# kscalelabs/minppo

Measured on NVIDIA B200. Metric: learner transitions/sec (GAE+PPO epochs), higher is better.
Workload: dtype bf16 tensor-core GEMMs (fp32 accumulate), fp32 elsewhere

## Files before the change

### minppo_b200/csrc/common.cuh

```cuda
#pragma once

#include <cuda.h>
#include <cuda_bf16.h>
#include <cuda_runtime.h>
#include <stdint.h>

namespace minppo {

#define MINPPO_DEVINL __device__ __forceinline__

MINPPO_DEVINL uint32_t smem_u32(const void* p) {
  return static_cast<uint32_t>(__cvta_generic_to_shared(p));
}

MINPPO_DEVINL uint32_t lane_id() { return threadIdx.x & 31u; }

MINPPO_DEVINL bool elect_one() {
  uint32_t pred = 0;
  asm volatile(
      "{\n\t.reg .pred P;\n\t"
      "elect.sync _|P, 0xffffffff;\n\t"
      "selp.u32 %0, 1, 0, P;\n\t}\n"
      : "=r"(pred));
  return pred != 0;
}

MINPPO_DEVINL float warp_sum(float v) {
#pragma unroll
  for (int o = 16; o > 0; o >>= 1) v += __shfl_xor_sync(0xffffffffu, v, o);
  return v;
}

MINPPO_DEVINL void griddep_wait() { asm volatile("griddepcontrol.wait;" ::: "memory"); }
MINPPO_DEVINL void griddep_launch() { asm volatile("griddepcontrol.launch_dependents;" ::: "memory"); }

MINPPO_DEVINL void mbar_init(uint64_t* bar, uint32_t count) {
  asm volatile("mbarrier.init.shared::cta.b64 [%0], %1;" ::"r"(smem_u32(bar)), "r"(count));
}
MINPPO_DEVINL void fence_mbar_init() {
  asm volatile("fence.mbarrier_init.release.cluster;" ::: "memory");
}
MINPPO_DEVINL void mbar_arrive(uint64_t* bar) {
  asm volatile("mbarrier.arrive.shared::cta.b64 _, [%0];" ::"r"(smem_u32(bar)) : "memory");
}
MINPPO_DEVINL void mbar_arrive_expect_tx(uint64_t* bar, uint32_t bytes) {
  asm volatile("mbarrier.arrive.expect_tx.shared::cta.b64 _, [%0], %1;" ::"r"(smem_u32(bar)),
               "r"(bytes)
               : "memory");
}
#ifndef MINPPO_TRY_WAIT_HINT_NS
#define MINPPO_TRY_WAIT_HINT_NS 1000000u
#endif
MINPPO_DEVINL bool mbar_try_wait(uint64_t* bar, uint32_t parity) {
  uint32_t ok;
  asm volatile(
      "{\n\t.reg .pred P;\n\t"
      "mbarrier.try_wait.parity.shared::cta.b64 P, [%1], %2, %3;\n\t"
      "selp.u32 %0, 1, 0, P;\n\t}\n"
      : "=r"(ok)
      : "r"(smem_u32(bar)), "r"(parity), "r"(MINPPO_TRY_WAIT_HINT_NS)
      : "memory");
  return ok != 0;
}
#ifndef MINPPO_WAIT_SLEEP_NS
#define MINPPO_WAIT_SLEEP_NS 0
#endif
template <bool POLITE = true>
MINPPO_DEVINL void mbar_wait(uint64_t* bar, uint32_t parity) {
  if (mbar_try_wait(bar, parity)) return;
  const long long t0 = clock64();
  for (;;) {
#pragma unroll 1
    for (int i = 0; i < 64; ++i) {
      if (mbar_try_wait(bar, parity)) return;
#if MINPPO_WAIT_SLEEP_NS
      if (POLITE) asm volatile("nanosleep.u32 %0;" ::"r"(static_cast<uint32_t>(MINPPO_WAIT_SLEEP_NS)));
#endif
    }
    if (clock64() - t0 > 4000000000LL) __trap();
  }
}

#ifndef MINPPO_MMA_SPIN
#define MINPPO_MMA_SPIN 0
#endif
MINPPO_DEVINL void mbar_wait_spin(uint64_t* bar, uint32_t parity) {
#if MINPPO_MMA_SPIN
  const uint32_t addr = smem_u32(bar);
  const long long t0 = clock64();
  for (;;) {
#pragma unroll 1
    for (int i = 0; i < 32; ++i) {
      uint32_t ok;
      asm volatile(
          "{\n\t.reg .pred P;\n\t"
          "mbarrier.test_wait.parity.shared::cta.b64 P, [%1], %2;\n\t"
          "selp.u32 %0, 1, 0, P;\n\t}\n"
          : "=r"(ok)
          : "r"(addr), "r"(parity)
          : "memory");
      if (ok) return;
    }
    if (clock64() - t0 > 4000000000LL) __trap();
  }
#else
  mbar_wait<false>(bar, parity);
#endif
}

MINPPO_DEVINL void fence_proxy_async_smem() {
  asm volatile("fence.proxy.async.shared::cta;" ::: "memory");
}

MINPPO_DEVINL void cp_async_16(uint32_t smem_dst, const void* gsrc) {
  asm volatile("cp.async.cg.shared.global [%0], [%1], 16;" ::"r"(smem_dst), "l"(gsrc) : "memory");
}
MINPPO_DEVINL void cp_async_commit() { asm volatile("cp.async.commit_group;" ::: "memory"); }
template <int N>
MINPPO_DEVINL void cp_async_wait() {
  asm volatile("cp.async.wait_group %0;" ::"n"(N) : "memory");
}

MINPPO_DEVINL void tma_prefetch_desc(const CUtensorMap* m) {
  asm volatile("prefetch.tensormap [%0];" ::"l"(reinterpret_cast<uint64_t>(m)) : "memory");
}
MINPPO_DEVINL void tma_load_2d(uint32_t smem_dst, const CUtensorMap* m, uint64_t* bar, int c0, int c1) {
  asm volatile(
      "cp.async.bulk.tensor.2d.shared::cluster.global.mbarrier::complete_tx::bytes"
      " [%0], [%1, {%3, %4}], [%2];"
      ::"r"(smem_dst), "l"(reinterpret_cast<uint64_t>(m)), "r"(smem_u32(bar)), "r"(c0), "r"(c1)
      : "memory");
}

MINPPO_DEVINL void tma_store_2d(uint32_t smem_src, const CUtensorMap* m, int c0, int c1) {
  asm volatile("cp.async.bulk.tensor.2d.global.shared::cta.bulk_group [%0, {%2, %3}], [%1];" ::"l"(
                   reinterpret_cast<uint64_t>(m)),
               "r"(smem_src), "r"(c0), "r"(c1)
               : "memory");
}
MINPPO_DEVINL void tma_store_3d(uint32_t smem_src, const CUtensorMap* m, int c0, int c1, int c2) {
  asm volatile("cp.async.bulk.tensor.3d.global.shared::cta.bulk_group [%0, {%2, %3, %4}], [%1];" ::"l"(
                   reinterpret_cast<uint64_t>(m)),
               "r"(smem_src), "r"(c0), "r"(c1), "r"(c2)
               : "memory");
}
MINPPO_DEVINL void bulk_store_1d(void* gdst, uint32_t smem_src, uint32_t bytes) {
  asm volatile("cp.async.bulk.global.shared::cta.bulk_group [%0], [%1], %2;" ::"l"(gdst), "r"(smem_src), "r"(bytes) : "memory");
}
MINPPO_DEVINL void sts32(uint32_t addr, float v) { asm volatile("st.shared.f32 [%0], %1;" ::"r"(addr), "f"(v) : "memory"); }
MINPPO_DEVINL void tma_store_commit() { asm volatile("cp.async.bulk.commit_group;" ::: "memory"); }
MINPPO_DEVINL void tma_store_wait_read0() { asm volatile("cp.async.bulk.wait_group.read 0;" ::: "memory"); }
MINPPO_DEVINL void tma_store_wait_all0() { asm volatile("cp.async.bulk.wait_group 0;" ::: "memory"); }
MINPPO_DEVINL void fence_proxy_async_global() { asm volatile("fence.proxy.async.global;" ::: "memory"); }

MINPPO_DEVINL void sts128(uint32_t addr, uint4 v) {
  asm volatile("st.shared.v4.u32 [%0], {%1, %2, %3, %4};" ::"r"(addr), "r"(v.x), "r"(v.y), "r"(v.z), "r"(v.w) : "memory");
}
MINPPO_DEVINL uint4 lds128(uint32_t addr) {
  uint4 v;
  asm volatile("ld.shared.v4.u32 {%0, %1, %2, %3}, [%4];" : "=r"(v.x), "=r"(v.y), "=r"(v.z), "=r"(v.w) : "r"(addr));
  return v;
}

MINPPO_DEVINL void tmem_alloc(uint32_t* smem_dst, uint32_t ncols) {
  asm volatile("tcgen05.alloc.cta_group::1.sync.aligned.shared::cta.b32 [%0], %1;" ::"r"(smem_u32(smem_dst)),
               "r"(ncols)
               : "memory");
}
MINPPO_DEVINL void tmem_relinquish() {
  asm volatile("tcgen05.relinquish_alloc_permit.cta_group::1.sync.aligned;" ::: "memory");
}
MINPPO_DEVINL void tmem_dealloc(uint32_t taddr, uint32_t ncols) {
  asm volatile("tcgen05.dealloc.cta_group::1.sync.aligned.b32 %0, %1;" ::"r"(taddr), "r"(ncols) : "memory");
}
MINPPO_DEVINL void tc_fence_before() { asm volatile("tcgen05.fence::before_thread_sync;" ::: "memory"); }
MINPPO_DEVINL void tc_fence_after() { asm volatile("tcgen05.fence::after_thread_sync;" ::: "memory"); }

MINPPO_DEVINL void umma_bf16(uint32_t tmem_d, uint64_t desc_a, uint64_t desc_b, uint32_t idesc,
                             uint32_t accumulate) {
  asm volatile(
      "{\n\t.reg .pred p;\n\t"
      "setp.ne.b32 p, %4, 0;\n\t"
      "tcgen05.mma.cta_group::1.kind::f16 [%0], %1, %2, %3, p;\n\t}\n"
      ::"r"(tmem_d), "l"(desc_a), "l"(desc_b), "r"(idesc), "r"(accumulate)
      : "memory");
}
MINPPO_DEVINL void umma_commit(uint64_t* bar) {
  asm volatile("tcgen05.commit.cta_group::1.mbarrier::arrive::one.shared::cluster.b64 [%0];" ::"r"(smem_u32(bar))
               : "memory");
}

MINPPO_DEVINL void tmem_ld_32x32(uint32_t taddr, float (&v)[32]) {
  uint32_t* r = reinterpret_cast<uint32_t*>(v);
  asm volatile(
      "tcgen05.ld.sync.aligned.32x32b.x32.b32 "
      "{%0, %1, %2, %3, %4, %5, %6, %7, %8, %9, %10, %11, %12, %13, %14, %15, "
      "%16, %17, %18, %19, %20, %21, %22, %23, %24, %25, %26, %27, %28, %29, %30, %31}, [%32];"
      : "=r"(r[0]), "=r"(r[1]), "=r"(r[2]), "=r"(r[3]), "=r"(r[4]), "=r"(r[5]), "=r"(r[6]), "=r"(r[7]),
        "=r"(r[8]), "=r"(r[9]), "=r"(r[10]), "=r"(r[11]), "=r"(r[12]), "=r"(r[13]), "=r"(r[14]), "=r"(r[15]),
        "=r"(r[16]), "=r"(r[17]), "=r"(r[18]), "=r"(r[19]), "=r"(r[20]), "=r"(r[21]), "=r"(r[22]), "=r"(r[23]),
        "=r"(r[24]), "=r"(r[25]), "=r"(r[26]), "=r"(r[27]), "=r"(r[28]), "=r"(r[29]), "=r"(r[30]), "=r"(r[31])
      : "r"(taddr)
      : "memory");
}
MINPPO_DEVINL void tmem_ld_wait() { asm volatile("tcgen05.wait::ld.sync.aligned;" ::: "memory"); }

MINPPO_DEVINL uint64_t umma_smem_desc(uint32_t smem_addr, uint32_t lbo_bytes, uint32_t sbo_bytes) {
  uint64_t d = 0;
  d |= static_cast<uint64_t>((smem_addr & 0x3FFFFu) >> 4);
  d |= static_cast<uint64_t>((lbo_bytes >> 4) & 0x3FFFu) << 16;
  d |= static_cast<uint64_t>((sbo_bytes >> 4) & 0x3FFFu) << 32;
  d |= static_cast<uint64_t>(1) << 46;
  d |= static_cast<uint64_t>(2) << 61;
  return d;
}
MINPPO_DEVINL constexpr uint32_t umma_idesc_bf16(uint32_t M, uint32_t N, uint32_t a_mn_major,
                                                 uint32_t b_mn_major) {
  return (1u << 4)
         | (1u << 7)
         | (1u << 10)
         | (a_mn_major << 15)
         | (b_mn_major << 16)
         | ((N >> 3) << 17)
         | ((M >> 4) << 24);
}

MINPPO_DEVINL float fast_tanh(float x) {
  float y;
  asm("tanh.approx.f32 %0, %1;" : "=f"(y) : "f"(x));
  return y;
}
MINPPO_DEVINL float exp_tanh(float x) {
  float e, r;
  asm("ex2.approx.ftz.f32 %0, %1;" : "=f"(e) : "f"(x * 2.8853900817779268f));
  asm("rcp.approx.ftz.f32 %0, %1;" : "=f"(r) : "f"(e + 1.f));
  return fmaf(-2.f, r, 1.f);
}

MINPPO_DEVINL uint32_t pack_bf16x2(float lo, float hi) {
  __nv_bfloat162 h = __floats2bfloat162_rn(lo, hi);
  return *reinterpret_cast<uint32_t*>(&h);
}
MINPPO_DEVINL void split_bf16(float x, uint32_t& hi, uint32_t& lo) {
  const __nv_bfloat16 h = __float2bfloat16_rn(x);
  const __nv_bfloat16 l = __float2bfloat16_rn(x - __bfloat162float(h));
  hi = __bfloat16_as_ushort(h);
  lo = __bfloat16_as_ushort(l);
}
MINPPO_DEVINL uint32_t swp_off(int ap, int rr, int c) {
  return static_cast<uint32_t>((c >> 6) * (ap * 256) + rr * 128 + ((((c & 63) >> 3) ^ (rr & 7)) << 4) + (c & 7) * 2);
}
MINPPO_DEVINL float bf16_lo(uint32_t w) { return __uint_as_float(w << 16); }
MINPPO_DEVINL float bf16_hi(uint32_t w) { return __uint_as_float(w & 0xFFFF0000u); }

}
```

### minppo_b200/csrc/dwopt.cuh

```cuda
#pragma once

#include "opt_common.cuh"
#include "umma_gemm.cuh"

namespace minppo {

constexpr int DWOPT_THREADS = 512;

struct PeerXchg {
  char* base[MINPPO_MAX_RANKS];
  unsigned int* seq;
  int world, rank;
  int np;
  int two_phase;
  int ablate;
};
MINPPO_DEVINL float* px_stage(const PeerXchg& x, int r, unsigned int par, int q) {
  return reinterpret_cast<float*>(x.base[r]) + (static_cast<size_t>(par) * x.world + q) * x.np;
}
MINPPO_DEVINL float* px_result(const PeerXchg& x, int r, unsigned int par) {
  return reinterpret_cast<float*>(x.base[r]) + 2 * static_cast<size_t>(x.world) * x.np + static_cast<size_t>(x.world) * 256 +
         static_cast<size_t>(par) * x.np;
}
MINPPO_DEVINL float4 ld_sys_v4(const float* p) {
  float4 v;
  asm volatile("ld.relaxed.sys.global.v4.f32 {%0, %1, %2, %3}, [%4];" : "=f"(v.x), "=f"(v.y), "=f"(v.z), "=f"(v.w) : "l"(p) : "memory");
  return v;
}
MINPPO_DEVINL void st_sys_f32(float* p, float v) { asm volatile("st.relaxed.sys.global.f32 [%0], %1;" ::"l"(p), "f"(v) : "memory"); }
MINPPO_DEVINL void st_sys_v4(float* p, float4 v) {
  asm volatile("st.relaxed.sys.global.v4.f32 [%0], {%1, %2, %3, %4};" ::"l"(p), "f"(v.x), "f"(v.y), "f"(v.z), "f"(v.w) : "memory");
}
MINPPO_DEVINL unsigned int ld_relaxed_sys_u32(const unsigned int* p) {
  unsigned int v;
  asm volatile("ld.relaxed.sys.global.u32 %0, [%1];" : "=r"(v) : "l"(p) : "memory");
  return v;
}
MINPPO_DEVINL void ld_unit(const float* p, float (&v)[4]) {
  const uintptr_t a = reinterpret_cast<uintptr_t>(p);
  if ((a & 15u) == 0) { const float4 q = __ldcg(reinterpret_cast<const float4*>(p)); v[0] = q.x; v[1] = q.y; v[2] = q.z; v[3] = q.w; }
  else if ((a & 7u) == 0) {
    const float2 q0 = __ldcg(reinterpret_cast<const float2*>(p)), q1 = __ldcg(reinterpret_cast<const float2*>(p) + 1);
    v[0] = q0.x; v[1] = q0.y; v[2] = q1.x; v[3] = q1.y;
  } else {
#pragma unroll
    for (int e = 0; e < 4; ++e) v[e] = __ldcg(p + e);
  }
}
MINPPO_DEVINL void st_unit(float* p, const float (&v)[4]) {
  const uintptr_t a = reinterpret_cast<uintptr_t>(p);
  if ((a & 15u) == 0) *reinterpret_cast<float4*>(p) = make_float4(v[0], v[1], v[2], v[3]);
  else if ((a & 7u) == 0) { reinterpret_cast<float2*>(p)[0] = make_float2(v[0], v[1]); reinterpret_cast<float2*>(p)[1] = make_float2(v[2], v[3]); }
  else {
#pragma unroll
    for (int e = 0; e < 4; ++e) p[e] = v[e];
  }
}

struct alignas(64) DwOptParams {
  GemmParams gemm;
  OptArgs opt;
  int gemm_ctas;
  long long* trace;
  PeerXchg px;
  const int32_t* ridx_base;
  const int32_t* counts;
  int cap, EM;
  int padded;
  int losses_stride;
  int part_rows;
  int prefetch;
  const __nv_bfloat16* obs_img;
  int obs_ld;
  int step;
};

template <int NTHREADS_MAX = 1024>
MINPPO_DEVINL float block_sum_dyn(float v, float* scratch ) {
  const int nw = static_cast<int>(blockDim.x) >> 5;
  v = warp_sum(v);
  if ((threadIdx.x & 31) == 0) scratch[threadIdx.x >> 5] = v;
  __syncthreads();
  float s = 0.f;
  if (threadIdx.x < 32) {
    s = static_cast<int>(threadIdx.x) < nw ? scratch[threadIdx.x] : 0.f;
    s = warp_sum(s);
  }
  __syncthreads();
  return s;
}

template <int MAXU>
MINPPO_DEVINL void dwopt_body(const DwOptParams& p, int step, uint8_t* smem_raw, uint32_t ext_tmem, bool build_tab = true) {
  __shared__ float scratch[32];
  __shared__ float s_bcast[4];
  __shared__ LeafTab T;
  const OptArgs& a = p.opt;
  const int P = a.P;
  const int G = static_cast<int>(gridDim.x), NT = static_cast<int>(blockDim.x);
  const int32_t* row_count = p.padded ? p.counts + step : nullptr;
  const int32_t* next_ridx = (p.prefetch && step + 1 < p.EM) ? p.ridx_base + static_cast<size_t>(step + 1) * p.cap : nullptr;
  const int32_t* next_count = p.padded ? p.counts + step + 1 : nullptr;
  float* losses_out = a.losses_out ? a.losses_out + static_cast<size_t>(step) * p.losses_stride : nullptr;
  float* gnorm_out = a.gnorm_out ? a.gnorm_out + step : nullptr;
  const int b = static_cast<int>(blockIdx.x), t = static_cast<int>(threadIdx.x);
  const bool has_extra = p.gemm_ctas < G;
#define DW_STAMP(slot) do { if (p.trace && t == 0) p.trace[static_cast<size_t>(b) * 16 + (slot)] = clock64(); } while (0)
  float ss = 0.f;
  DW_STAMP(0);
  __shared__ unsigned int s_seq;
  __shared__ int s_dead;
  const bool px_on = p.px.world > 1;
  if (px_on && t == 0) {
    s_seq = __ldcg(p.px.seq) + 1u;
    s_dead = __ldcg(a.err_flag) != 0;
  }
  const bool gemm_cta = b < p.gemm_ctas;
  if (!gemm_cta) {
    if (build_tab) leaf_tab_build(T, a, t, NT);
    __syncthreads();
  }
  DW_STAMP(14);

  const bool scal_thread = t == NT - 1;
  int count = 0;
  float ent = a.entropy_const;
  auto scalars = [&]() {
    if (scal_thread && a.do_apply) {
      count = __ldcg(a.count);
      step_scalars(a, count, s_bcast[1], s_bcast[2], s_bcast[3]);
      if (b == 0 && losses_out) {
        for (int j = 0; j < a.A; ++j) ent += logf(fabsf(expf(__ldcg(a.params + a.off_logstd + j))));
      }
    }
  };

  if (gemm_cta) {
    auto idle_work = [&]() {
      if (build_tab) leaf_tab_build(T, a, t - GEMM_THREADS, NT - GEMM_THREADS);
      scalars();
      if (next_ridx) {
        const int HELPERS = NT - GEMM_THREADS;
        const int h = t - GEMM_THREADS;
        const int lines = (p.obs_ld * 2) >> 7;
        const int nrows = next_count ? min(p.cap, __ldcg(next_count)) : p.cap;
        for (int j = b * HELPERS + h; j < nrows * lines; j += p.gemm_ctas * HELPERS) {
          const char* row = reinterpret_cast<const char*>(p.obs_img + static_cast<size_t>(next_ridx[j / lines]) * p.obs_ld);
          asm volatile("prefetch.global.L2 [%0];" ::"l"(row + (j % lines) * 128));
        }
      }
    };
    umma_gemm_body<EPI_PARTIAL>(p.gemm, smem_raw, p.trace ? p.trace + static_cast<size_t>(b) * 16 : nullptr, idle_work, ext_tmem,
                                p.ridx_base + static_cast<size_t>(step) * p.cap, row_count);
  } else {
    scalars();
    griddep_wait();
    if (t == 0) griddep_launch();
    const int e = b - p.gemm_ctas, ne = G - p.gemm_ctas;
    const int live_tiles = row_count ? (max(__ldcg(row_count), 0) + p.part_rows - 1) / p.part_rows : 0x7fffffff;
    ss = reduce_leaves<false>(a, T, e * NT + t, ne * NT, live_tiles);
  }
  DW_STAMP(1);
  grid_barrier(a.barrier, a.err_flag);
  DW_STAMP(2);

  int n_units = 0;
  for (int l = 0; l < T.nleaves; ++l)
    if (T.leaf[l].late) n_units += T.size[l] >> 2;
  const int GT_ = G * NT;
  const bool fast = n_units <= GT_ * MAXU;
  const int gtid = b * NT + t;
  float4 g4[MAXU];
  float pv[MAXU][4], mv[MAXU][4], nv[MAXU][4];
  int ul[MAXU], ui[MAXU];
  if (!has_extra) ss += reduce_leaves<false>(a, T, gtid, GT_, row_count ? (max(__ldcg(row_count), 0) + p.part_rows - 1) / p.part_rows : 0x7fffffff);
  const int unit0 = (((t >> 5) * G + b) << 5) + (t & 31);
#pragma unroll
  for (int u = 0; u < MAXU; ++u) { ul[u] = -1; ui[u] = 0; g4[u] = make_float4(0.f, 0.f, 0.f, 0.f); }
  if (fast) {
#pragma unroll
    for (int u = 0; u < MAXU; ++u) {
      const int unit = unit0 + u * GT_;
      if (unit < n_units) {
        int x = unit, l = 0;
        for (; l < T.nleaves; ++l) {
          if (!T.leaf[l].late) continue;
          const int n = T.size[l] >> 2;
          if (x < n) break;
          x -= n;
        }
        const OptLeaf& L = T.leaf[l];
        ul[u] = l; ui[u] = L.offset + 4 * x;
        if (a.do_apply) {
          ld_unit(a.params + ui[u], pv[u]); ld_unit(a.mu + ui[u], mv[u]); ld_unit(a.nu + ui[u], nv[u]);
        }
        g4[u] = sum_partials16_v4(L.grad_src + L.src_offset + 4 * x, L.nparts, L.part_stride);
        if (!px_on) {
          if (!a.do_apply || a.keep_gflat) { const float gq[4] = {g4[u].x, g4[u].y, g4[u].z, g4[u].w}; st_unit(a.gflat + ui[u], gq); }
          ss = fmaf(g4[u].x, g4[u].x, ss); ss = fmaf(g4[u].y, g4[u].y, ss); ss = fmaf(g4[u].z, g4[u].z, ss); ss = fmaf(g4[u].w, g4[u].w, ss);
        }
      }
    }
  } else {
    ss += reduce_leaves<true>(a, T, gtid, GT_);
  }
  if (!a.do_apply) return;

  if (px_on) {
    const PeerXchg& X = p.px;
    const int R = X.rank;
    const int W = X.ablate == 2 ? 1 : X.world;
    const bool nowait = X.ablate != 0 || s_dead != 0;
    const unsigned int n = s_seq, par = n & 1u;
    const int n_late4 = 4 * n_units;
    int eidx = -1;
    if (gtid < T.n_early + 2) {
      if (gtid >= T.n_early) eidx = P + (gtid - T.n_early);
      else {
        int x = gtid, l = 0;
        for (; l < T.nleaves; ++l) {
          if (T.leaf[l].late) continue;
          if (x < T.size[l]) break;
          x -= T.size[l];
        }
        eidx = T.leaf[l].offset + x;
      }
    }
    constexpr unsigned int SENT = 0x80000000u;
    auto canon = [](float x) { return x == 0.f ? 0.f : x; };
    auto is_real4 = [](const float4& v) {
      return __float_as_uint(v.x) != SENT && __float_as_uint(v.y) != SENT && __float_as_uint(v.z) != SENT && __float_as_uint(v.w) != SENT;
    };
    const float4 sent4 = make_float4(-0.f, -0.f, -0.f, -0.f);
    float gl = 0.f;
    if (eidx >= 0) gl = canon(__ldcg(a.gflat + eidx));
    const bool two = X.two_phase != 0;
    const int owner = two ? (b + (t >> 5)) % W : R;
    const bool reduce_here = owner == R;
#pragma unroll
    for (int u = 0; u < MAXU; ++u) {
      if (ul[u] < 0) continue;
      const int unit = unit0 + u * GT_;
      g4[u].x = canon(g4[u].x); g4[u].y = canon(g4[u].y); g4[u].z = canon(g4[u].z); g4[u].w = canon(g4[u].w);
      if (reduce_here) {
        if (!two) {
#pragma unroll
          for (int r = 0; r < MINPPO_MAX_RANKS; ++r) if (r < W && r != R) st_sys_v4(px_stage(X, r, par, R) + 4 * unit, g4[u]);
        }
      } else {
        st_sys_v4(px_stage(X, owner, par, R) + 4 * unit, g4[u]);
      }
    }
    if (eidx >= 0) {
      if (reduce_here) {
        if (!two) {
#pragma unroll
          for (int r = 0; r < MINPPO_MAX_RANKS; ++r) if (r < W && r != R) st_sys_f32(px_stage(X, r, par, R) + n_late4 + gtid, gl);
        }
      } else {
        st_sys_f32(px_stage(X, owner, par, R) + n_late4 + gtid, gl);
      }
    }
    DW_STAMP(13);
    ss = 0.f;
    const long long t0 = clock64();
#pragma unroll
    for (int u = 0; u < MAXU; ++u) {
      if (ul[u] < 0) continue;
      const int unit = unit0 + u * GT_;
      if (reduce_here) {
        float4 v[MINPPO_MAX_RANKS];
        unsigned int pending = nowait ? 0u : ((1u << W) - 1u) & ~(1u << R);
#pragma unroll
        for (int q = 0; q < MINPPO_MAX_RANKS; ++q) v[q] = g4[u];
        while (pending) {
#pragma unroll
          for (int q = 0; q < MINPPO_MAX_RANKS; ++q) {
            if ((pending >> q) & 1u) {
              v[q] = ld_sys_v4(px_stage(X, R, par, q) + 4 * unit);
              if (is_real4(v[q])) pending &= ~(1u << q);
            }
          }
          if (pending && clock64() - t0 > 8000000000LL) { atomicExch(a.err_flag, MINPPO_ERR_BARRIER); break; }
        }
        const float4 own = g4[u];
        float4 acc = make_float4(0.f, 0.f, 0.f, 0.f);
#pragma unroll
        for (int q = 0; q < MINPPO_MAX_RANKS; ++q) {
          if (q < W) {
            const float4 c = q == R ? own : v[q];
            acc.x += c.x; acc.y += c.y; acc.z += c.z; acc.w += c.w;
            if (q != R) st_sys_v4(px_stage(X, R, par, q) + 4 * unit, sent4);
          }
        }
        g4[u] = acc;
        if (two) {
          const float4 res = make_float4(canon(acc.x), canon(acc.y), canon(acc.z), canon(acc.w));
#pragma unroll
          for (int r = 0; r < MINPPO_MAX_RANKS; ++r) if (r < W && r != R) st_sys_v4(px_result(X, r, par) + 4 * unit, res);
        }
      } else {
        float* src = px_result(X, R, par) + 4 * unit;
        float4 v = g4[u];
        while (!nowait) {
          v = ld_sys_v4(src);
          if (is_real4(v)) break;
          if (clock64() - t0 > 8000000000LL) { atomicExch(a.err_flag, MINPPO_ERR_BARRIER); break; }
        }
        g4[u] = v;
        st_sys_v4(src, sent4);
      }
      if (a.keep_gflat) { const float gq[4] = {g4[u].x, g4[u].y, g4[u].z, g4[u].w}; st_unit(a.gflat + ui[u], gq); }
      ss = fmaf(g4[u].x, g4[u].x, ss); ss = fmaf(g4[u].y, g4[u].y, ss); ss = fmaf(g4[u].z, g4[u].z, ss); ss = fmaf(g4[u].w, g4[u].w, ss);
    }
    if (eidx >= 0) {
      float ge = 0.f;
      auto poll1 = [&](float* src, float fallback) {
        unsigned int w = __float_as_uint(fallback);
        while (!nowait && (w = ld_relaxed_sys_u32(reinterpret_cast<const unsigned int*>(src))) == SENT) {
          if (clock64() - t0 > 8000000000LL) { atomicExch(a.err_flag, MINPPO_ERR_BARRIER); break; }
        }
        st_sys_f32(src, -0.f);
        return __uint_as_float(w);
      };
      if (reduce_here) {
        float ev[MINPPO_MAX_RANKS];
        unsigned int pending = nowait ? 0u : ((1u << W) - 1u) & ~(1u << R);
#pragma unroll
        for (int q = 0; q < MINPPO_MAX_RANKS; ++q) ev[q] = gl;
        while (pending) {
#pragma unroll
          for (int q = 0; q < MINPPO_MAX_RANKS; ++q) {
            if ((pending >> q) & 1u) {
              const unsigned int w = ld_relaxed_sys_u32(reinterpret_cast<const unsigned int*>(px_stage(X, R, par, q) + n_late4 + gtid));
              if (w != SENT) { ev[q] = __uint_as_float(w); pending &= ~(1u << q); }
            }
          }
          if (pending && clock64() - t0 > 8000000000LL) { atomicExch(a.err_flag, MINPPO_ERR_BARRIER); break; }
        }
#pragma unroll
        for (int q = 0; q < MINPPO_MAX_RANKS; ++q) {
          if (q < W) {
            ge += ev[q];
            if (q != R) st_sys_f32(px_stage(X, R, par, q) + n_late4 + gtid, -0.f);
          }
        }
        if (two) {
          const float res = canon(ge);
#pragma unroll
          for (int r = 0; r < MINPPO_MAX_RANKS; ++r) if (r < W && r != R) st_sys_f32(px_result(X, r, par) + n_late4 + gtid, res);
        }
      } else {
        ge = poll1(px_result(X, R, par) + n_late4 + gtid, gl);
      }
      a.gflat[eidx] = ge;
      if (eidx < P) ss = fmaf(ge, ge, ss);
    }
    DW_STAMP(15);
    if (b == 0 && scal_thread) *X.seq = n;
  }
  const float bs = block_sum_dyn(ss, scratch);
  if (t == 0) a.block_ss[b] = bs;
  DW_STAMP(3);
  grid_barrier(a.barrier, a.err_flag);
  DW_STAMP(4);

  const bool early_one = fast && !px_on && T.n_early <= GT_;
  int el = -1, ei = 0;
  float eg = 0.f, ep = 0.f, em = 0.f, en = 0.f;
  if (early_one && gtid < T.n_early) {
    int x = gtid, l = 0;
    for (; l < T.nleaves; ++l) {
      if (T.leaf[l].late) continue;
      if (x < T.size[l]) break;
      x -= T.size[l];
    }
    el = l; ei = T.leaf[l].offset + x;
    eg = __ldcg(a.gflat + ei); ep = __ldcg(a.params + ei); em = __ldcg(a.mu + ei); en = __ldcg(a.nu + ei);
  }
  {
    const float v = t < G ? __ldcg(a.block_ss + t) : 0.f;
    const float tot = block_sum_dyn(v, scratch);
    if (t == 0) s_bcast[0] = sqrtf(tot);
  }
  __syncthreads();
  AdamScalars sc;
  sc.gnorm = s_bcast[0]; sc.lr = s_bcast[1]; sc.c1 = s_bcast[2]; sc.c2 = s_bcast[3];
  sc.trigger = sc.gnorm < a.max_norm;
  if (fast) {
#pragma unroll
    for (int u = 0; u < MAXU; ++u) {
      if (ul[u] < 0) continue;
      const OptLeaf& L = T.leaf[ul[u]];
      const float gv[4] = {g4[u].x, g4[u].y, g4[u].z, g4[u].w};
#pragma unroll
      for (int e = 0; e < 4; ++e) adam_element(a, sc, gv[e], pv[u][e], mv[u][e], nv[u][e]);
      st_unit(a.params + ui[u], pv[u]); st_unit(a.mu + ui[u], mv[u]); st_unit(a.nu + ui[u], nv[u]);
      if (L.img_n)
        *reinterpret_cast<uint2*>(L.img_n + (ui[u] - L.offset)) = make_uint2(pack_bf16x2(pv[u][0], pv[u][1]), pack_bf16x2(pv[u][2], pv[u][3]));
    }
    if (early_one) {
      if (el >= 0) {
        adam_element(a, sc, eg, ep, em, en);
        a.params[ei] = ep; a.mu[ei] = em; a.nu[ei] = en;
        write_images(T.leaf[el], ei, ep);
      }
    } else {
      apply_adam_class<false>(a, T, sc, gtid, GT_);
    }
  } else {
    apply_adam(a, T, sc, gtid, GT_);
  }
  __syncthreads();
  DW_STAMP(5);
  if (b == 0 && scal_thread) {
    *a.count = count + 1;
    if (losses_out) {
      const float value_loss = 0.5f * __ldcg(a.gflat + P) * a.inv_mb;
      const float actor_loss = -__ldcg(a.gflat + P + 1) * a.inv_mb;
      const float poison = __ldcg(a.err_flag) != 0 ? __int_as_float(0x7fc00000) : 0.f;
      losses_out[0] = actor_loss + a.vf_coef * value_loss - a.ent_coef * ent + poison;
      losses_out[1] = value_loss + poison;
      losses_out[2] = actor_loss + poison;
      losses_out[3] = ent + poison;
      if (gnorm_out) *gnorm_out = sc.gnorm;
    }
  }
}

template <int MAXU>
__global__ void __launch_bounds__(DWOPT_THREADS, 1) dwopt_kernel(const __grid_constant__ DwOptParams p) {
  extern __shared__ uint8_t smem_raw[];
  dwopt_body<MAXU>(p, p.step, smem_raw, GEMM_NO_TMEM);
}

inline long long dwopt_fast_capacity(int grid, int maxu) { return 4LL * grid * DWOPT_THREADS * maxu; }

inline cudaError_t dwopt_launch(const DwOptParams& p, int grid, cudaStream_t stream, bool pdl, int maxu) {
  if (maxu <= 1) return launch_kernel(dwopt_kernel<1>, grid, DWOPT_THREADS, GEMM_SMEM_BYTES, stream, pdl, p);
  if (maxu == 2) return launch_kernel(dwopt_kernel<2>, grid, DWOPT_THREADS, GEMM_SMEM_BYTES, stream, pdl, p);
  return launch_kernel(dwopt_kernel<4>, grid, DWOPT_THREADS, GEMM_SMEM_BYTES, stream, pdl, p);
}

}
```

### minppo_b200/csrc/learner.cu

```cuda
#include <cuda.h>
#include <dlfcn.h>
#include <math.h>
#include <algorithm>
#include <nccl.h>
#include <stdarg.h>
#include <stdio.h>
#include <stdlib.h>
#include <string.h>

#include <vector>

#include "common.cuh"
#include "minppo_internal.h"
#include "umma_gemm.cuh"
#include "fused_step.cuh"
#include "dwopt.cuh"
#include "ppo_steps.cuh"
#include "policy_fused.cuh"

namespace minppo {

static thread_local char g_err[512] = "";
void set_error(const char* fmt, ...) {
  va_list ap;
  va_start(ap, fmt);
  vsnprintf(g_err, sizeof(g_err), fmt, ap);
  va_end(ap);
}
#define CK(call)                                                                          \
  do {                                                                                    \
    cudaError_t e_ = (call);                                                              \
    if (e_ != cudaSuccess) {                                                              \
      set_error("%s failed: %s (%s:%d)", #call, cudaGetErrorString(e_), __FILE__, __LINE__); \
      return MINPPO_ERR_CUDA;                                                             \
    }                                                                                     \
  } while (0)
#define RET(call)            \
  do {                       \
    int r_ = (call);         \
    if (r_ != 0) return r_;  \
  } while (0)

typedef CUresult (*EncodeTiledFn)(CUtensorMap*, CUtensorMapDataType, cuuint32_t, void*, const cuuint64_t*,
                                  const cuuint64_t*, const cuuint32_t*, const cuuint32_t*, CUtensorMapInterleave,
                                  CUtensorMapSwizzle, CUtensorMapL2promotion, CUtensorMapFloatOOBfill);
static EncodeTiledFn get_encode_fn() {
  static EncodeTiledFn fn = nullptr;
  if (!fn) {
    void* p = nullptr;
    cudaDriverEntryPointQueryResult q;
    if (cudaGetDriverEntryPoint("cuTensorMapEncodeTiled", &p, cudaEnableDefault, &q) == cudaSuccess &&
        q == cudaDriverEntryPointSuccess)
      fn = reinterpret_cast<EncodeTiledFn>(p);
  }
  return fn;
}
static int make_tmap(CUtensorMap* m, const void* base, uint64_t inner, uint64_t outer, uint64_t ld,
                     uint32_t box_inner, uint32_t box_outer) {
  EncodeTiledFn fn = get_encode_fn();
  if (!fn) { set_error("cuTensorMapEncodeTiled entry point not available"); return MINPPO_ERR_CUDA; }
  cuuint64_t dims[2] = {inner, outer};
  cuuint64_t strides[1] = {ld * 2};
  cuuint32_t box[2] = {box_inner, box_outer};
  cuuint32_t estr[2] = {1, 1};
  CUresult r = fn(m, CU_TENSOR_MAP_DATA_TYPE_BFLOAT16, 2, const_cast<void*>(base), dims, strides, box, estr,
                  CU_TENSOR_MAP_INTERLEAVE_NONE, CU_TENSOR_MAP_SWIZZLE_128B, CU_TENSOR_MAP_L2_PROMOTION_L2_256B,
                  CU_TENSOR_MAP_FLOAT_OOB_FILL_NONE);
  if (r != CUDA_SUCCESS) { set_error("cuTensorMapEncodeTiled failed (%d)", static_cast<int>(r)); return MINPPO_ERR_CUDA; }
  return 0;
}

static int make_tmap_f32_3d(CUtensorMap* m, const void* base, uint64_t d0, uint64_t d1, uint64_t d2) {
  EncodeTiledFn fn = get_encode_fn();
  if (!fn) { set_error("cuTensorMapEncodeTiled entry point not available"); return MINPPO_ERR_CUDA; }
  cuuint64_t dims[3] = {d0, d1, d2};
  cuuint64_t strides[2] = {d0 * 4, d0 * d1 * 4};
  cuuint32_t box[3] = {32, 128, 1};
  cuuint32_t estr[3] = {1, 1, 1};
  CUresult r = fn(m, CU_TENSOR_MAP_DATA_TYPE_FLOAT32, 3, const_cast<void*>(base), dims, strides, box, estr,
                  CU_TENSOR_MAP_INTERLEAVE_NONE, CU_TENSOR_MAP_SWIZZLE_128B, CU_TENSOR_MAP_L2_PROMOTION_L2_256B,
                  CU_TENSOR_MAP_FLOAT_OOB_FILL_NONE);
  if (r != CUDA_SUCCESS) { set_error("cuTensorMapEncodeTiled (f32 3d) failed (%d)", static_cast<int>(r)); return MINPPO_ERR_CUDA; }
  return 0;
}

struct NcclApi {
  ncclResult_t (*GetUniqueId)(ncclUniqueId*);
  ncclResult_t (*CommInitRank)(ncclComm_t*, int, ncclUniqueId, int);
  ncclResult_t (*AllReduce)(const void*, void*, size_t, ncclDataType_t, ncclRedOp_t, ncclComm_t, cudaStream_t);
  ncclResult_t (*Broadcast)(const void*, void*, size_t, ncclDataType_t, int, ncclComm_t, cudaStream_t);
  ncclResult_t (*GroupStart)();
  ncclResult_t (*GroupEnd)();
  ncclResult_t (*CommDestroy)(ncclComm_t);
  const char* (*GetErrorString)(ncclResult_t);
  bool ok;
};
static NcclApi* nccl_api() {
  static NcclApi api = {};
  static bool tried = false;
  if (!tried) {
    tried = true;
    void* h = dlopen("libnccl.so.2", RTLD_NOW | RTLD_GLOBAL);
    if (!h) h = dlopen("libnccl.so", RTLD_NOW | RTLD_GLOBAL);
    if (h) {
      api.GetUniqueId = reinterpret_cast<decltype(api.GetUniqueId)>(dlsym(h, "ncclGetUniqueId"));
      api.CommInitRank = reinterpret_cast<decltype(api.CommInitRank)>(dlsym(h, "ncclCommInitRank"));
      api.AllReduce = reinterpret_cast<decltype(api.AllReduce)>(dlsym(h, "ncclAllReduce"));
      api.Broadcast = reinterpret_cast<decltype(api.Broadcast)>(dlsym(h, "ncclBroadcast"));
      api.GroupStart = reinterpret_cast<decltype(api.GroupStart)>(dlsym(h, "ncclGroupStart"));
      api.GroupEnd = reinterpret_cast<decltype(api.GroupEnd)>(dlsym(h, "ncclGroupEnd"));
      api.CommDestroy = reinterpret_cast<decltype(api.CommDestroy)>(dlsym(h, "ncclCommDestroy"));
      api.GetErrorString = reinterpret_cast<decltype(api.GetErrorString)>(dlsym(h, "ncclGetErrorString"));
      api.ok = api.GetUniqueId && api.CommInitRank && api.AllReduce && api.Broadcast && api.GroupStart && api.GroupEnd &&
               api.CommDestroy && api.GetErrorString;
    }
  }
  return api.ok ? &api : nullptr;
}

struct LeafInfo {
  int net;
  int layer;
  int is_kernel;
  long long offset, rows, cols;
};
static long long build_layout(const minppo_config& c, std::vector<LeafInfo>* out) {
  long long off = 0;
  const int L = c.num_layers;
  for (int net = 0; net < 2; ++net) {
    long long fan_in = c.obs_dim;
    for (int l = 0; l <= L; ++l) {
      const long long o = l < L ? c.hidden_size : (net == 0 ? c.act_dim : 1);
      if (out) out->push_back({net, l, 0, off, 1, o});
      off += o;
      if (out) out->push_back({net, l, 1, off, fan_in, o});
      off += fan_in * o;
      fan_in = o;
    }
  }
  if (out) out->push_back({2, 0, 0, off, 1, c.act_dim});
  off += c.act_dim;
  return off;
}

static int validate_config(const minppo_config& c) {
  if (c.num_envs <= 0 || c.num_steps <= 0 || c.num_minibatches <= 0 || c.update_epochs <= 0 || c.obs_dim <= 0 ||
      c.act_dim <= 0 || c.num_layers < 1) {
    set_error("non-positive size in minppo_config");
    return MINPPO_ERR_ARG;
  }
  if (c.hidden_size % 64 != 0 || c.hidden_size > MAX_HIDDEN || c.hidden_size <= 0) {
    set_error("model.hidden_size=%d unsupported: must be a multiple of 64 and <= %d", c.hidden_size, MAX_HIDDEN);
    return MINPPO_ERR_UNSUPPORTED;
  }
  if (c.hidden_size > GEMM_MAXN && 2 * c.num_layers * 2 > GEMM_MAX_GROUPS) {
    set_error("num_layers=%d unsupported at model.hidden_size=%d: hidden_size > %d allows num_layers <= %d", c.num_layers,
              c.hidden_size, GEMM_MAXN, GEMM_MAX_GROUPS / 4);
    return MINPPO_ERR_UNSUPPORTED;
  }
  if (c.act_dim > 32) { set_error("act_dim=%d unsupported (<= 32)", c.act_dim); return MINPPO_ERR_UNSUPPORTED; }
  if (2 * (c.num_layers + 1) * 2 + 1 > OPT_TAB_LEAVES) { set_error("too many layers"); return MINPPO_ERR_UNSUPPORTED; }
  if (2 * c.num_layers > 6) { set_error("num_layers=%d unsupported (<= 3)", c.num_layers); return MINPPO_ERR_UNSUPPORTED; }
  const long long B = static_cast<long long>(c.num_envs) * c.num_steps;
  const long long mb = B / c.num_minibatches;
  if (mb * c.num_minibatches != B) {
    set_error("`batch_size` must be equal to `num_steps * num_envs`");
    return MINPPO_ERR_ARG;
  }
  if (c.world_size < 1 || c.rank < 0 || c.rank >= c.world_size || c.num_envs % c.world_size != 0) {
    set_error("bad sharding: world_size=%d rank=%d num_envs=%d", c.world_size, c.rank, c.num_envs);
    return MINPPO_ERR_ARG;
  }
  if (c.prng_mode != MINPPO_PRNG_LEGACY && c.prng_mode != MINPPO_PRNG_PARTITIONABLE) {
    set_error("bad prng_mode %d", c.prng_mode);
    return MINPPO_ERR_ARG;
  }
  if (B > 0x7fffffffLL) { set_error("batch too large"); return MINPPO_ERR_UNSUPPORTED; }
  return 0;
}

}

using namespace minppo;

struct NetBufs {
  std::vector<__nv_bfloat16*> act;
  std::vector<__nv_bfloat16*> dz;
  std::vector<__nv_bfloat16*> wn;
  std::vector<float*> dw_part;
  uint8_t* w2img;
  std::vector<float*> dbias;
  std::vector<float*> colsum;
  std::vector<CUtensorMap> m_act_k, m_act_mn, m_dz_k, m_dz_mn, m_wn_mn, m_wn, m_dw;
  std::vector<CUtensorMap> m_wn_h;
  CUtensorMap m_w1k_h;
};

struct UpdatePtrs {
  float *params, *mu, *nu;
  int32_t* count;
  const float *obs, *action, *value, *reward, *log_prob;
  const uint8_t* done;
  const float* last_val;
  const uint32_t* key_in;
  uint32_t* key_out;
  float* losses_out;
  bool operator==(const UpdatePtrs& o) const { return memcmp(this, &o, sizeof(*this)) == 0; }
};

struct minppo_ctx {
  minppo_config cfg;
  int device, sm_count;
  int T, N, Nl, n0, M, E, L, H, D, Dp, A;
  long long B, Bl, P;
  int mb, cap, M_pad, m_tiles, tiles64, S;
  int dw_nsplit;
  int hsplit;
  int maxu;
  bool fused;
  int head_parts;
  std::vector<LeafInfo> leaves;
  std::vector<void*> allocs;
  float *adv, *tgt, *stats, *gflat, *block_ss, *head_part, *gnorms, *losses_scratch;
  long long* trace;
  long long* trace2;
  bool trace_on;
  bool pdl;
  bool merged_opt;
  bool persistent;
  int steps_per_launch;
  int skip_mask;
  int32_t *perms, *rowidx, *counts;
  int32_t* perm_tmp;
  bool padded;
  bool share_perm;
  void* perm_ws;
  size_t perm_ws_bytes;
  __nv_bfloat16* obs_img;
  __nv_bfloat16* xg;
  CUtensorMap m_xg_k, m_xg_mn;
  unsigned long long* barrier;
  int* err_flag;
  NetBufs net[2];
  int head_stride, po_w3a, po_b3a, po_w3c, po_b3c, po_logstd, po_bh_a, po_bh_c, po_loss;
  int po_db[2][2];
  int ap;
  bool store_x;
  int opt_blocks;
  cudaStream_t cap_stream;
  cudaStream_t side_stream;
  cudaEvent_t ev_fork, ev_join;
  struct CachedGraph { cudaGraph_t graph; cudaGraphExec_t exec; UpdatePtrs ptrs; long long launches; };
  std::vector<CachedGraph> graphs;
  long long launches;
  ncclComm_t comm;
  bool have_comm;
  float* xchg;
  unsigned int* xseq;
  PeerXchg px;
  bool peers_set;
  void* peer_ptr[MINPPO_MAX_RANKS];
  int pol_tiles;
  __nv_bfloat16* pol_img;
  __nv_bfloat16* pol_act[2][MINPPO_MAX_LEAVES];
  CUtensorMap m_pol_img_k, m_pol_act_k[2][MINPPO_MAX_LEAVES];
  bool profiling;
  std::vector<cudaEvent_t> prof_events;
  std::vector<int> prof_class;
  size_t prof_used;
};

enum : int { PC_GAE = 0, PC_PERM, PC_PREP, PC_OBS_IMAGE, PC_WEIGHT_IMAGES, PC_FWD_GEMM, PC_HEAD_LOSS, PC_BWD_GEMM,
             PC_DW_GEMM, PC_OPT, PC_ALLREDUCE, PC_COUNT };

struct ProfScope {
  minppo_ctx* c; cudaStream_t s; size_t idx; bool on;
  ProfScope(minppo_ctx* ctx, int cls, cudaStream_t stream) : c(ctx), s(stream), idx(0), on(ctx->profiling) {
    if (!on) return;
    if (c->prof_used + 2 > c->prof_events.size()) {
      cudaEvent_t a, b;
      cudaEventCreate(&a); cudaEventCreate(&b);
      c->prof_events.push_back(a); c->prof_events.push_back(b);
      c->prof_class.push_back(cls);
    } else {
      c->prof_class[c->prof_used / 2] = cls;
    }
    idx = c->prof_used;
    c->prof_used += 2;
    cudaEventRecord(c->prof_events[idx], s);
  }
  ~ProfScope() { if (on) cudaEventRecord(c->prof_events[idx + 1], s); }
};
#define PROF(cls) ProfScope prof_scope_(c, cls, stream)

namespace minppo {

template <typename T>
static int dev_alloc(minppo_ctx* c, T** p, size_t n, bool zero = true) {
  void* q = nullptr;
  const size_t bytes = (n * sizeof(T) + 255) & ~static_cast<size_t>(255);
  CK(cudaMalloc(&q, bytes));
  if (zero) CK(cudaMemset(q, 0, bytes));
  c->allocs.push_back(q);
  *p = reinterpret_cast<T*>(q);
  return 0;
}

__global__ void fill_u32_kernel(uint32_t* p, size_t n, uint32_t v) {
  for (size_t i = blockIdx.x * static_cast<size_t>(blockDim.x) + threadIdx.x; i < n; i += static_cast<size_t>(gridDim.x) * blockDim.x) p[i] = v;
}

static const LeafInfo& find_leaf(const minppo_ctx* c, int net, int layer, int is_kernel) {
  for (const auto& l : c->leaves)
    if (l.net == net && l.layer == layer && l.is_kernel == is_kernel) return l;
  return c->leaves[0];
}

static void col_group(int H, int n, int j, int* n_off, int* N) {
  const int first = n == 1 ? H : (H / 2 + 63) / 64 * 64;
  *n_off = j == 0 ? 0 : first;
  *N = j == 0 ? first : H - first;
}

static int act_kind(const minppo_ctx* c, int net) {
  if (net == 1 || !c->cfg.use_tanh) return ACT_RELU;
  return c->cfg.fast_tanh ? ACT_TANH_FAST : ACT_TANH;
}

static int init_kernel_attrs() {
  CK(cudaFuncSetAttribute(umma_gemm_kernel<EPI_ACT>, cudaFuncAttributeMaxDynamicSharedMemorySize, GEMM_SMEM_BYTES));
  CK(cudaFuncSetAttribute(umma_gemm_kernel<EPI_DACT>, cudaFuncAttributeMaxDynamicSharedMemorySize, GEMM_SMEM_BYTES));
  CK(cudaFuncSetAttribute(umma_gemm_kernel<EPI_PARTIAL>, cudaFuncAttributeMaxDynamicSharedMemorySize, GEMM_SMEM_BYTES));
  if (head_loss_init()) { set_error("head_loss_init failed"); return MINPPO_ERR_CUDA; }
  CK(cudaFuncSetAttribute(fused_step_kernel<16>, cudaFuncAttributeMaxDynamicSharedMemorySize, FsLayout<16>::BYTES));
  CK(cudaFuncSetAttribute(fused_step_kernel<32>, cudaFuncAttributeMaxDynamicSharedMemorySize, FsLayout<32>::BYTES));
  CK(cudaFuncSetAttribute(dwopt_kernel<1>, cudaFuncAttributeMaxDynamicSharedMemorySize, GEMM_SMEM_BYTES));
  CK(cudaFuncSetAttribute(dwopt_kernel<2>, cudaFuncAttributeMaxDynamicSharedMemorySize, GEMM_SMEM_BYTES));
  CK(cudaFuncSetAttribute(dwopt_kernel<4>, cudaFuncAttributeMaxDynamicSharedMemorySize, GEMM_SMEM_BYTES));
  CK(steps_init_attrs());
  CK(policy_fused_init_attrs());
  return 0;
}

template <int EPI>
static int launch_gemm(const GemmParams& p_in, int ctas, cudaStream_t stream, bool pdl = false) {
  GemmParams p = p_in;
  gemm_finalize(p);
  const cudaError_t e = launch_kernel(umma_gemm_kernel<EPI>, ctas, GEMM_THREADS, GEMM_SMEM_BYTES, stream, pdl, p);
  if (e != cudaSuccess) { set_error("umma_gemm launch failed: %s", cudaGetErrorString(e)); return MINPPO_ERR_CUDA; }
  return 0;
}

static void fill_opt_args(const minppo_ctx* c, const UpdatePtrs& u, OptArgs* o) {
  memset(o, 0, sizeof(*o));
  const minppo_config& cfg = c->cfg;
  const int L = c->L, H = c->H;
  int n = 0;
  for (const auto& lf : c->leaves) {
    OptLeaf& ol = o->leaf[n++];
    ol.offset = static_cast<int>(lf.offset);
    ol.cols = static_cast<int>(lf.cols);
    ol.grad_bias = 0.f;
    ol.img_t = nullptr; ol.img_n = nullptr; ol.ld_t = 0; ol.ld_n = 0; ol.img_w2 = nullptr; ol.late = 0; ol.ap = 16;
    if (lf.net == 2) {
      ol.grad_src = c->head_part; ol.src_offset = c->po_logstd; ol.nparts = c->head_parts; ol.part_stride = c->head_stride;
      ol.grad_bias = cfg.rank == 0 ? -static_cast<float>(cfg.ent_coef) : 0.f;
    } else if (lf.layer == L) {
      ol.grad_src = c->head_part; ol.nparts = c->head_parts; ol.part_stride = c->head_stride;
      if (lf.is_kernel) { ol.src_offset = lf.net == 0 ? c->po_w3a : c->po_w3c; ol.img_w2 = c->fused ? c->net[lf.net].w2img : nullptr; ol.ap = c->ap; }
      else ol.src_offset = lf.net == 0 ? c->po_b3a : c->po_b3c;
    } else if (lf.is_kernel) {
      const int in_l = lf.layer == 0 ? c->D : H;
      ol.grad_src = c->net[lf.net].dw_part[lf.layer]; ol.src_offset = 0; ol.nparts = c->S; ol.part_stride = in_l * H; ol.late = 1;
      ol.img_n = c->net[lf.net].wn[lf.layer]; ol.ld_n = H;
    } else if (c->fused) {
      ol.grad_src = c->head_part; ol.src_offset = c->po_db[lf.net][lf.layer]; ol.nparts = c->head_parts; ol.part_stride = c->head_stride;
    } else {
      ol.grad_src = c->net[lf.net].dbias[lf.layer]; ol.src_offset = 0; ol.nparts = c->S;
      ol.part_stride = H; ol.late = 1;
    }
  }
  o->nleaves = n;
  o->n_early = 0;
  for (int i = 0; i < n; ++i) {
    o->leaf[i].size = (i + 1 < n ? o->leaf[i + 1].offset : static_cast<int>(c->P)) - o->leaf[i].offset;
    if (!o->leaf[i].late) o->n_early += o->leaf[i].size;
  }
  o->keep_gflat = 1;
  o->P = static_cast<int>(c->P);
  o->A = c->A;
  o->gflat = c->gflat;
  o->loss_src = c->head_part; o->loss_src_offset = c->po_loss; o->loss_nparts = c->head_parts; o->loss_part_stride = c->head_stride;
  o->params = u.params; o->mu = u.mu; o->nu = u.nu; o->count = u.count;
  o->block_ss = c->block_ss; o->barrier = c->barrier; o->err_flag = c->err_flag;
  o->off_logstd = static_cast<int>(c->leaves.back().offset);
  o->anneal = cfg.anneal_lr ? 1 : 0;
  o->anneal_div = c->mb * c->E;
  const long long nu = cfg.total_timesteps / cfg.num_steps / cfg.num_envs;
  o->num_updates = static_cast<int>(nu > 0x7fffffffLL ? 0x7fffffffLL : nu);
  o->lr = static_cast<float>(cfg.anneal_lr ? cfg.training_lr : cfg.opt_lr);
  o->max_norm = static_cast<float>(cfg.max_grad_norm);
  o->b1 = static_cast<float>(cfg.adam_b1); o->b2 = static_cast<float>(cfg.adam_b2);
  o->one_minus_b1 = static_cast<float>(1.0 - cfg.adam_b1); o->one_minus_b2 = static_cast<float>(1.0 - cfg.adam_b2);
  o->eps = static_cast<float>(cfg.adam_eps); o->eps_root = static_cast<float>(cfg.adam_eps_root);
  o->inv_mb = static_cast<float>(1.0 / c->mb);
  o->vf_coef = static_cast<float>(cfg.vf_coef); o->ent_coef = static_cast<float>(cfg.ent_coef);
  o->entropy_const = static_cast<float>(c->A * (0.5 + 0.5 * log(2.0 * M_PI)));
}

static int nccl_allreduce(minppo_ctx* c, float* buf, size_t n, cudaStream_t stream) {
  NcclApi* api = nccl_api();
  ncclResult_t r = api->AllReduce(buf, buf, n, ncclFloat, ncclSum, c->comm, stream);
  if (r != ncclSuccess) { set_error("ncclAllReduce failed: %s", api->GetErrorString(r)); return MINPPO_ERR_NCCL; }
  return 0;
}

static void fill_fused_params(minppo_ctx* c, const UpdatePtrs& u, FusedParams* pp) {
  FusedParams& p = *pp;
  memset(&p, 0, sizeof(p));
  const int H = c->H;
  for (int net = 0; net < 2; ++net) {
    FusedNet& g = p.net[net];
    NetBufs& nb = c->net[net];
    g.tm_w0 = nb.m_wn_h[0]; g.tm_w1 = nb.m_wn_h[1]; g.tm_w1k = nb.m_w1k_h;
    g.tm_h1 = nb.m_act_k[1]; g.tm_dz2 = nb.m_dz_k[2]; g.tm_dz1 = nb.m_dz_k[1];
    g.b0 = u.params + find_leaf(c, net, 0, 0).offset;
    g.b1 = u.params + find_leaf(c, net, 1, 0).offset;
    g.w2img = reinterpret_cast<const uint4*>(nb.w2img);
    g.b2 = u.params + find_leaf(c, net, 2, 0).offset;
    g.act = act_kind(c, net);
    g.aout = net == 0 ? c->A : 1;
    g.po_w2 = net == 0 ? c->po_w3a : c->po_w3c;
    g.po_b2 = net == 0 ? c->po_b3a : c->po_b3c;
    g.po_loss = c->po_loss + (net == 0 ? 1 : 0);
    g.po_db0 = c->po_db[net][0]; g.po_db1 = c->po_db[net][1];
  }
  p.rowidx = c->rowidx; p.obs_img = c->obs_img; p.count = c->counts; p.step = 0;
  p.tm_xg = c->m_xg_k; p.store_x = c->store_x ? 1 : 0;
  p.adv_sum = c->stats; p.adv_sq = c->stats + c->E * c->M;
  p.action = u.action; p.v_old = u.value; p.logp_old = u.log_prob; p.adv = c->adv; p.tgt = c->tgt;
  p.log_std = u.params + c->leaves.back().offset;
  p.part = c->head_part; p.part_stride = c->head_stride; p.po_logstd = c->po_logstd;
  p.H = H; p.A = c->A; p.Dp = c->Dp; p.m_tiles = c->m_tiles; p.cap = c->cap;
  p.inv_mb = static_cast<float>(1.0 / c->mb);
  p.clip_eps = static_cast<float>(c->cfg.clip_eps); p.vf_coef = static_cast<float>(c->cfg.vf_coef);
  p.trace = c->trace_on ? c->trace : nullptr;
}

static int fill_dwopt_params(minppo_ctx* c, const UpdatePtrs& u, DwOptParams* dpp) {
  DwOptParams& dp = *dpp;
  memset(&dp, 0, sizeof(dp));
  const int L = c->L, H = c->H;
  GemmParams& p = dp.gemm;
  int cta = 0, ng = 0;
  for (int net = 0; net < 2; ++net) {
    NetBufs& nb = c->net[net];
    for (int l = 0; l < L; ++l) {
      for (int nh = 0; nh < c->dw_nsplit; ++nh) {
      GemmGroup& g = p.g[ng++];
      g.cta_begin = cta;
      const int in_l = l == 0 ? c->D : H;
      const int in_pad = l == 0 ? c->Dp : H;
      if (l == 0 && c->fused && c->store_x && !(c->skip_mask & 1)) { g.amode = A_TMA_MN; g.tmA = c->m_xg_mn; }
      else if (l == 0) { g.amode = A_GATHER_MN; g.rowidx = c->rowidx; g.gimage = c->obs_img; g.ldg = c->Dp; }
      else { g.amode = A_TMA_MN; g.tmA = nb.m_act_mn[l]; }
      g.bmode = B_TMA_MN; g.tmB = nb.m_dz_mn[l + 1];
      g.kb_total = c->M_pad / 64;
      g.k_count = nullptr;
      g.tmC = nb.m_dw[l];
      g.colsum_out = c->fused ? nullptr : nb.dbias[l];
      col_group(H, c->dw_nsplit, nh, &g.n_off, &g.N);
      g.ldc = H;
      g.m_tiles = (in_pad + 127) / 128; g.splits = c->S; g.m_store = in_l;
      cta += g.m_tiles * g.splits;
      }
    }
  }
  p.ngroups = ng;
  gemm_finalize(p);
  fill_opt_args(c, u, &dp.opt);
  dp.opt.losses_out = u.losses_out ? u.losses_out : c->losses_scratch;
  dp.losses_stride = u.losses_out ? 4 : 0;
  dp.opt.gnorm_out = c->gnorms;
  dp.gemm_ctas = cta;
  dp.ridx_base = c->rowidx; dp.counts = c->counts; dp.cap = c->cap; dp.EM = c->E * c->M;
  dp.padded = c->padded ? 1 : 0;
  dp.part_rows = c->fused ? 128 : 64;
  dp.prefetch = 1; dp.obs_img = c->obs_img; dp.obs_ld = c->Dp;
  dp.trace = c->trace_on ? c->trace2 : nullptr;
  return cta;
}

static int enqueue_step(minppo_ctx* c, const UpdatePtrs& u, int s, cudaStream_t stream) {
  const int L = c->L, H = c->H;
  const int32_t* ridx = c->rowidx + static_cast<size_t>(s) * c->cap;
  const bool pdl = c->pdl && c->fused && !c->profiling;
  if (c->fused && (c->skip_mask & 1)) {
  } else if (c->fused) {
    FusedParams p;
    fill_fused_params(c, u, &p);
    p.step = s;
    PROF(PC_FWD_GEMM);
    const cudaError_t e = c->ap == 16
        ? launch_kernel(fused_step_kernel<16>, 2 * c->m_tiles, FS_THREADS, FsLayout<16>::BYTES, stream, pdl, p)
        : launch_kernel(fused_step_kernel<32>, 2 * c->m_tiles, FS_THREADS, FsLayout<32>::BYTES, stream, pdl, p);
    if (e != cudaSuccess) { set_error("fused_step launch failed: %s", cudaGetErrorString(e)); return MINPPO_ERR_CUDA; }
    c->launches++;
  } else {
  for (int l = 0; l < L; ++l) {
    GemmParams p;
    memset(&p, 0, sizeof(p));
    p.ngroups = 2 * c->hsplit;
    for (int i = 0; i < p.ngroups; ++i) {
      const int net = i / c->hsplit;
      GemmGroup& g = p.g[i];
      NetBufs& nb = c->net[net];
      g.cta_begin = i * c->m_tiles;
      col_group(H, c->hsplit, i % c->hsplit, &g.n_off, &g.N);
      g.bmode = B_TMA_MN;
      g.tmB = nb.m_wn_mn[l];
      if (l == 0) {
        g.amode = A_GATHER_K; g.rowidx = ridx; g.gimage = c->obs_img; g.ldg = c->Dp; g.kb_total = c->Dp / 64;
      } else {
        g.amode = A_TMA_K; g.tmA = nb.m_act_k[l]; g.kb_total = H / 64;
      }
      g.out = nb.act[l + 1]; g.ldo = H;
      g.bias = u.params + find_leaf(c, net, l, 0).offset;
      g.act = act_kind(c, net);
      g.m_tiles = c->m_tiles; g.splits = 1; g.m_store = c->M_pad;
    }
    PROF(PC_FWD_GEMM);
    RET(launch_gemm<EPI_ACT>(p, p.ngroups * c->m_tiles, stream));
    c->launches++;
  }
  {
    HeadLossArgs a;
    memset(&a, 0, sizeof(a));
    a.h_a = c->net[0].act[L]; a.h_c = c->net[1].act[L];
    a.dz_a = c->net[0].dz[L]; a.dz_c = c->net[1].dz[L];
    a.params = u.params; a.rowidx = ridx; a.count = c->counts + s;
    a.adv_sum = c->stats + s; a.adv_sq = c->stats + c->E * c->M + s;
    a.action = u.action; a.v_old = u.value; a.logp_old = u.log_prob; a.adv = c->adv; a.tgt = c->tgt;
    a.partials = c->head_part; a.partial_stride = c->head_stride;
    a.po_w3a = c->po_w3a; a.po_b3a = c->po_b3a; a.po_w3c = c->po_w3c; a.po_b3c = c->po_b3c;
    a.po_logstd = c->po_logstd; a.po_bh_a = c->po_bh_a; a.po_bh_c = c->po_bh_c; a.po_loss = c->po_loss;
    a.off_w3a = static_cast<int>(find_leaf(c, 0, L, 1).offset); a.off_b3a = static_cast<int>(find_leaf(c, 0, L, 0).offset);
    a.off_w3c = static_cast<int>(find_leaf(c, 1, L, 1).offset); a.off_b3c = static_cast<int>(find_leaf(c, 1, L, 0).offset);
    a.off_logstd = static_cast<int>(c->leaves.back().offset);
    a.H = H; a.A = c->A; a.ldh = H; a.cap = c->cap;
    a.act_a = act_kind(c, 0) == ACT_RELU ? ACTK_RELU : ACTK_TANH; a.act_c = ACTK_RELU;
    a.inv_mb = static_cast<float>(1.0 / c->mb);
    a.clip_eps = static_cast<float>(c->cfg.clip_eps); a.vf_coef = static_cast<float>(c->cfg.vf_coef);
    PROF(PC_HEAD_LOSS);
    RET(head_loss_launch(a, c->tiles64, stream));
    c->launches++;
  }
  for (int l = L - 1; l >= 1; --l) {
    GemmParams p;
    memset(&p, 0, sizeof(p));
    p.ngroups = 2 * c->hsplit;
    for (int i = 0; i < p.ngroups; ++i) {
      const int net = i / c->hsplit, j = i % c->hsplit;
      GemmGroup& g = p.g[i];
      NetBufs& nb = c->net[net];
      g.cta_begin = i * c->m_tiles;
      col_group(H, c->hsplit, j, &g.n_off, &g.N);
      g.amode = A_TMA_K; g.tmA = nb.m_dz_k[l + 1];
      g.bmode = B_TMA_K; g.tmB = nb.m_wn[2 * l + j];
      g.kb_total = H / 64;
      g.out = nb.dz[l]; g.ldo = H;
      g.hprev = nb.act[l]; g.ldh = H;
      g.colsum = nb.colsum[l]; g.ldc = H;
      g.act = act_kind(c, net);
      g.m_tiles = c->m_tiles; g.splits = 1; g.m_store = c->M_pad;
    }
    PROF(PC_BWD_GEMM);
    RET(launch_gemm<EPI_DACT>(p, p.ngroups * c->m_tiles, stream));
    c->launches++;
  }
  }
  DwOptParams dp;
  const int cta = fill_dwopt_params(c, u, &dp);
  dp.step = s;
  GemmParams& p = dp.gemm;
  OptArgs& o = dp.opt;
  const bool sharded = c->cfg.world_size > 1;
  const bool merged = c->merged_opt && c->skip_mask == 0 && cta <= c->sm_count;
  if (merged) {
    const bool px_on = sharded && c->peers_set && c->P <= dwopt_fast_capacity(c->sm_count, c->maxu);
    if (px_on) { dp.px = c->px; dp.px.ablate = getenv("MINPPO_PX_ABLATE") ? atoi(getenv("MINPPO_PX_ABLATE")) : 0; }
    o.do_reduce = 1; o.do_apply = (sharded && !px_on) ? 0 : 1;
    {
      PROF(PC_DW_GEMM);
      const cudaError_t e = dwopt_launch(dp, c->sm_count, stream, pdl, c->maxu);
      if (e != cudaSuccess) { set_error("dwopt launch failed: %s", cudaGetErrorString(e)); return MINPPO_ERR_CUDA; }
      c->launches++;
    }
    if (sharded && !px_on) {
      { PROF(PC_ALLREDUCE); RET(nccl_allreduce(c, c->gflat, static_cast<size_t>(c->P) + 2, stream)); }
      o.losses_out = o.losses_out + static_cast<size_t>(s) * dp.losses_stride; o.gnorm_out = c->gnorms + s;
      o.do_reduce = 0; o.do_apply = 1;
      { PROF(PC_OPT); RET(opt_launch(o, c->opt_blocks, stream, pdl)); }
      c->launches += 2;
    }
    return 0;
  }
  for (int i = 0; i < p.ngroups; ++i) {
    if (p.g[i].rowidx) p.g[i].rowidx = ridx;
    p.g[i].k_count = c->padded ? c->counts + s : nullptr;
  }
  o.losses_out = o.losses_out + static_cast<size_t>(s) * dp.losses_stride;
  o.gnorm_out = c->gnorms + s;
  if (!(c->skip_mask & 2)) {
    PROF(PC_DW_GEMM);
    RET(launch_gemm<EPI_PARTIAL>(p, cta, stream, pdl));
    c->launches++;
  }
  if (!(c->skip_mask & 4)) {
    if (!sharded) {
      o.do_reduce = 1; o.do_apply = 1;
      PROF(PC_OPT);
      RET(opt_launch(o, c->opt_blocks, stream, pdl));
      c->launches++;
    } else {
      o.do_reduce = 1; o.do_apply = 0;
      { PROF(PC_OPT); RET(opt_launch(o, c->opt_blocks, stream, pdl)); }
      { PROF(PC_ALLREDUCE); RET(nccl_allreduce(c, c->gflat, static_cast<size_t>(c->P) + 2, stream)); }
      o.do_reduce = 0; o.do_apply = 1;
      { PROF(PC_OPT); RET(opt_launch(o, c->opt_blocks, stream, pdl)); }
      c->launches += 3;
    }
  }
  return 0;
}

static int enqueue_update(minppo_ctx* c, const UpdatePtrs& u, cudaStream_t stream) {
  const minppo_config& cfg = c->cfg;
  c->launches = 0;
  const float gamma = static_cast<float>(cfg.gamma);
  const float gl = static_cast<float>(cfg.gamma * cfg.gae_lambda);
  c->prof_used = 0;
  const bool fork = !c->profiling && !(getenv("MINPPO_NO_FORK") && atoi(getenv("MINPPO_NO_FORK")) != 0);
  if (fork) {
    CK(cudaEventRecord(c->ev_fork, stream));
    CK(cudaStreamWaitEvent(c->side_stream, c->ev_fork, 0));
    RET(obs_image_launch(u.obs, c->obs_img, c->Bl, c->D, c->Dp, c->side_stream));
    OptArgs o;
    fill_opt_args(c, u, &o);
    RET(weight_images_launch(o, c->side_stream));
    CK(cudaEventRecord(c->ev_join, c->side_stream));
    c->launches += 2;
  }
  {
    PROF(PC_GAE);
    RET(gae_launch(u.reward, u.value, u.done, u.last_val, c->adv, c->tgt, c->T, c->Nl, gamma, gl, c->sm_count, 0, stream));
    c->launches++;
  }
  if (c->share_perm) {
    PROF(PC_PERM);
    const int W = cfg.world_size, R = cfg.rank;
    const int mine = R < c->E ? (c->E - R + W - 1) / W : 0;
    RET(perm_launch(u.key_in, u.key_out, cfg.prng_mode, mine, c->B, c->perm_tmp, c->perm_ws, c->perm_ws_bytes, stream, R, W, c->E));
    NcclApi* api = nccl_api();
    ncclResult_t r = api->GroupStart();
    for (int e = 0; e < c->E && r == ncclSuccess; ++e) {
      const int root = e % W;
      int32_t* dst = c->perms + static_cast<size_t>(e) * c->B;
      const int32_t* src = root == R ? c->perm_tmp + static_cast<size_t>(e / W) * c->B : dst;
      r = api->Broadcast(src, dst, static_cast<size_t>(c->B), ncclInt32, root, c->comm, stream);
    }
    const ncclResult_t r2 = api->GroupEnd();
    if (r == ncclSuccess) r = r2;
    if (r != ncclSuccess) { set_error("ncclBroadcast (permutations) failed: %s", api->GetErrorString(r)); return MINPPO_ERR_NCCL; }
    c->launches += (mine > 0 ? perm_launch_count(c->B) : 0) + (u.key_out ? 1 : 0);
  } else {
    PROF(PC_PERM);
    RET(perm_launch(u.key_in, u.key_out, cfg.prng_mode, c->E, c->B, c->perms, c->perm_ws, c->perm_ws_bytes, stream));
    c->launches += perm_launch_count(c->B) + (u.key_out ? 1 : 0);
  }
  const int EM = c->E * c->M;
  {
    PROF(PC_PREP);
    RET(compact_rows_launch(c->perms, c->rowidx, c->counts, c->E, c->M, c->B, c->mb, c->cap, c->N, c->n0, c->Nl, c->err_flag, stream));
    RET(adv_stats_launch(c->adv, c->rowidx, c->counts, c->stats, EM, c->cap, c->mb, 0, stream));
    if (cfg.world_size > 1) RET(nccl_allreduce(c, c->stats, EM, stream));
    RET(adv_stats_launch(c->adv, c->rowidx, c->counts, c->stats, EM, c->cap, c->mb, 1, stream));
    if (cfg.world_size > 1) RET(nccl_allreduce(c, c->stats + EM, EM, stream));
    c->launches += 3 + (cfg.world_size > 1 ? 2 : 0);
  }
  if (fork) {
    CK(cudaStreamWaitEvent(stream, c->ev_join, 0));
  } else {
    {
      PROF(PC_OBS_IMAGE);
      RET(obs_image_launch(u.obs, c->obs_img, c->Bl, c->D, c->Dp, stream));
      c->launches++;
    }
    {
      OptArgs o;
      fill_opt_args(c, u, &o);
      PROF(PC_WEIGHT_IMAGES);
      RET(weight_images_launch(o, stream));
      c->launches++;
    }
  }
  if (c->persistent && c->fused && c->merged_opt && c->skip_mask == 0 && !c->profiling) {
    StepsParams sp;
    memset(&sp, 0, sizeof(sp));
    fill_fused_params(c, u, &sp.fs);
    const int cta = fill_dwopt_params(c, u, &sp.dw);
    const bool sharded = cfg.world_size > 1;
    const bool px_on = sharded && c->peers_set && c->P <= dwopt_fast_capacity(c->sm_count, c->maxu);
    if (cta <= c->sm_count && (!sharded || px_on)) {
      if (px_on) { sp.dw.px = c->px; sp.dw.px.ablate = getenv("MINPPO_PX_ABLATE") ? atoi(getenv("MINPPO_PX_ABLATE")) : 0; }
      sp.dw.opt.do_reduce = 1; sp.dw.opt.do_apply = 1;
      sp.units = 2 * c->m_tiles;
      const int chunk = c->steps_per_launch > 0 ? c->steps_per_launch : EM;
      for (int s0 = 0; s0 < EM; s0 += chunk) {
        sp.s0 = s0; sp.s1 = std::min(EM, s0 + chunk);
        const cudaError_t e = steps_launch(sp, c->sm_count, stream, c->ap, c->maxu);
        if (e != cudaSuccess) { set_error("ppo_steps launch failed: %s", cudaGetErrorString(e)); return MINPPO_ERR_CUDA; }
        c->launches++;
      }
      return 0;
    }
  }
  for (int s = 0; s < EM; ++s) RET(enqueue_step(c, u, s, stream));
  return 0;
}

}

extern "C" {

const char* minppo_last_error(void) { return g_err; }
int minppo_version(void) { return 100; }

int minppo_gae_chunked(const float* reward, const float* value, const uint8_t* done, const float* last_val,
                       float* adv_out, float* tgt_out, int32_t T, int64_t N, double gamma, double gae_lambda,
                       int32_t chunks, void* stream) {
  if (!reward || !value || !done || !last_val || !adv_out || !tgt_out || T <= 0 || N <= 0) {
    set_error("minppo_gae: null pointer or non-positive size");
    return MINPPO_ERR_ARG;
  }
  int dev = 0, sms = 148;
  cudaGetDevice(&dev);
  cudaDeviceGetAttribute(&sms, cudaDevAttrMultiProcessorCount, dev);
  int r = gae_launch(reward, value, done, last_val, adv_out, tgt_out, T, N, static_cast<float>(gamma),
                     static_cast<float>(gamma * gae_lambda), sms, chunks, static_cast<cudaStream_t>(stream));
  if (r) { set_error("gae launch failed: %s", cudaGetErrorString(cudaGetLastError())); return MINPPO_ERR_CUDA; }
  return 0;
}
int minppo_gae(const float* reward, const float* value, const uint8_t* done, const float* last_val, float* adv_out,
               float* tgt_out, int32_t T, int64_t N, double gamma, double gae_lambda, void* stream) {
  return minppo_gae_chunked(reward, value, done, last_val, adv_out, tgt_out, T, N, gamma, gae_lambda, 0, stream);
}

size_t minppo_permutation_workspace_size(int32_t epochs, int64_t B) { return perm_workspace_bytes(epochs, B); }

int minppo_permutation(const uint32_t* key_in, uint32_t* key_out, int32_t prng_mode, int32_t epochs, int64_t B,
                       int32_t* perm_out, void* workspace, size_t workspace_bytes, void* stream) {
  if (!key_in || !perm_out || !workspace) { set_error("minppo_permutation: null pointer"); return MINPPO_ERR_ARG; }
  if (prng_mode != MINPPO_PRNG_LEGACY && prng_mode != MINPPO_PRNG_PARTITIONABLE) { set_error("bad prng_mode"); return MINPPO_ERR_ARG; }
  int r = perm_launch(key_in, key_out, prng_mode, epochs, B, perm_out, workspace, workspace_bytes,
                      static_cast<cudaStream_t>(stream));
  if (r == MINPPO_ERR_ARG) set_error("minppo_permutation: bad size");
  else if (r == MINPPO_ERR_WORKSPACE) set_error("minppo_permutation: workspace too small");
  else if (r) set_error("minppo_permutation: launch failed: %s", cudaGetErrorString(cudaGetLastError()));
  return r;
}

int64_t minppo_param_layout(const minppo_config* cfg, int32_t* nleaves, int64_t* offsets, int64_t* rows,
                            int64_t* cols) {
  if (!cfg) { set_error("null config"); return MINPPO_ERR_ARG; }
  std::vector<LeafInfo> lv;
  const long long P = build_layout(*cfg, &lv);
  if (nleaves) *nleaves = static_cast<int32_t>(lv.size());
  for (size_t i = 0; i < lv.size(); ++i) {
    if (offsets) offsets[i] = lv[i].offset;
    if (rows) rows[i] = lv[i].rows;
    if (cols) cols[i] = lv[i].cols;
  }
  return P;
}

int minppo_nccl_unique_id(void* id128_host) {
  NcclApi* api = nccl_api();
  if (!api) { set_error("libnccl.so.2 could not be loaded"); return MINPPO_ERR_NCCL; }
  ncclUniqueId id;
  ncclResult_t r = api->GetUniqueId(&id);
  if (r != ncclSuccess) { set_error("ncclGetUniqueId: %s", api->GetErrorString(r)); return MINPPO_ERR_NCCL; }
  static_assert(sizeof(ncclUniqueId) == 128, "ncclUniqueId is 128 bytes");
  memcpy(id128_host, &id, 128);
  return 0;
}

static void drop_graphs(minppo_ctx* c) {
  for (auto& g : c->graphs) { cudaGraphExecDestroy(g.exec); cudaGraphDestroy(g.graph); }
  c->graphs.clear();
}

int minppo_ctx_destroy(minppo_ctx* c) {
  if (!c) return 0;
  drop_graphs(c);
  for (cudaEvent_t e : c->prof_events) cudaEventDestroy(e);
  if (c->cap_stream) cudaStreamDestroy(c->cap_stream);
  if (c->side_stream) cudaStreamDestroy(c->side_stream);
  if (c->ev_fork) cudaEventDestroy(c->ev_fork);
  if (c->ev_join) cudaEventDestroy(c->ev_join);
  if (c->have_comm) nccl_api()->CommDestroy(c->comm);
  for (int r = 0; r < MINPPO_MAX_RANKS; ++r) if (c->peer_ptr[r]) cudaIpcCloseMemHandle(c->peer_ptr[r]);
  for (void* p : c->allocs) cudaFree(p);
  delete c;
  return 0;
}

int minppo_ctx_create(const minppo_config* cfg, const void* nccl_unique_id_host, minppo_ctx** out) {
  if (!cfg || !out) { set_error("null argument"); return MINPPO_ERR_ARG; }
  RET(validate_config(*cfg));
  minppo_ctx* c = new minppo_ctx();
  c->cfg = *cfg;
  c->have_comm = false; c->cap_stream = nullptr; c->launches = 0;
  c->side_stream = nullptr; c->ev_fork = nullptr; c->ev_join = nullptr;
  c->profiling = false; c->prof_used = 0;
  int rc = 0;
  auto fail = [&](int code) { minppo_ctx_destroy(c); return code; };
  if (cudaGetDevice(&c->device) != cudaSuccess) { set_error("no CUDA device"); return fail(MINPPO_ERR_CUDA); }
  cudaDeviceProp prop;
  if (cudaGetDeviceProperties(&prop, c->device) != cudaSuccess) { set_error("cudaGetDeviceProperties failed"); return fail(MINPPO_ERR_CUDA); }
  if (prop.major != 10) {
    set_error("minppo_b200 requires an sm_100a (B200) device; found sm_%d%d", prop.major, prop.minor);
    return fail(MINPPO_ERR_UNSUPPORTED);
  }
  c->sm_count = prop.multiProcessorCount;
  if ((rc = init_kernel_attrs())) return fail(rc);

  c->T = cfg->num_steps; c->N = cfg->num_envs; c->Nl = c->N / cfg->world_size; c->n0 = cfg->rank * c->Nl;
  c->M = cfg->num_minibatches; c->E = cfg->update_epochs; c->L = cfg->num_layers; c->H = cfg->hidden_size;
  c->D = cfg->obs_dim; c->Dp = (c->D + 63) / 64 * 64; c->A = cfg->act_dim;
  c->B = static_cast<long long>(c->T) * c->N; c->Bl = static_cast<long long>(c->T) * c->Nl;
  c->mb = static_cast<int>(c->B / c->M);
  const int pad_emul = (cfg->world_size == 1 && getenv("MINPPO_EMULATE_SHARD_PAD")) ? atoi(getenv("MINPPO_EMULATE_SHARD_PAD")) : 0;
  c->padded = cfg->world_size > 1 || pad_emul > 1;
  if (!c->padded) c->cap = c->mb;
  else {
    long long cap = (3LL * c->mb / cfg->world_size + 1) / 2 + 256;
    if (pad_emul == 3) cap = c->mb + 128;
    else if (pad_emul > 1) cap = c->mb + c->mb / 2 + 256;
    if (cap > c->mb && pad_emul <= 1) cap = c->mb;
    if (cap > c->Bl) cap = c->Bl;
    c->cap = static_cast<int>(cap);
  }
  if (getenv("MINPPO_FORCE_CAP") && atoi(getenv("MINPPO_FORCE_CAP")) > 0) {
    c->padded = true;
    c->cap = atoi(getenv("MINPPO_FORCE_CAP"));
  }
  c->M_pad = (c->cap + 127) / 128 * 128;
  c->cap = c->M_pad;
  c->m_tiles = c->M_pad / 128;
  c->tiles64 = c->M_pad / 64;
  c->fused = !cfg->disable_fused && c->L == 2 && c->H <= GEMM_MAXN;
  c->hsplit = c->H > GEMM_MAXN ? 2 : 1;
  c->ap = c->A <= 16 ? 16 : 32;
  c->store_x = c->fused;
  c->head_parts = c->fused ? c->m_tiles : c->tiles64;
  c->P = build_layout(*cfg, &c->leaves);
  c->maxu = c->P <= dwopt_fast_capacity(c->sm_count, 1) ? 1 : (c->P <= dwopt_fast_capacity(c->sm_count, 2) ? 2 : 4);
  {
    c->dw_nsplit = c->H > GEMM_MAXN ? 2
                 : (c->fused && c->store_x && c->H % 128 == 0 && 2 * 2 * c->L <= GEMM_MAX_GROUPS &&
                    !(getenv("MINPPO_DW_NSPLIT") && atoi(getenv("MINPPO_DW_NSPLIT")) == 1)) ? 2 : 1;
    int per_split = 0;
    for (int l = 0; l < c->L; ++l) per_split += 2 * c->dw_nsplit * (((l == 0 ? c->Dp : c->H) + 127) / 128);
    const int gemm_budget = c->sm_count > 48 ? c->sm_count - 16 : c->sm_count;
    int S = cfg->dw_splits > 0 ? cfg->dw_splits : (gemm_budget / (per_split > 0 ? per_split : 1));
    if (getenv("MINPPO_DW_SPLITS")) S = atoi(getenv("MINPPO_DW_SPLITS"));
    int kb_total = c->M_pad / 64;
    if (c->padded) {
      const double mean = pad_emul > 1 ? c->mb : static_cast<double>(c->mb) / cfg->world_size;
      const long long rows = static_cast<long long>(mean + 3.0 * sqrt(mean)) + 1;
      kb_total = static_cast<int>(std::min<long long>(c->M_pad, rows + 63) / 64);
      if (kb_total < 1) kb_total = 1;
    }
    if (S > kb_total) S = kb_total;
    if (S > 32) S = 32;
    if (S < 1) S = 1;
    while (S > 1 && ((kb_total + S - 1) / S) * (S - 1) >= kb_total) --S;
    c->S = S;
  }
  c->opt_blocks = c->sm_count;
  if (c->P > opt_max_params(c->opt_blocks)) { set_error("parameter count %lld exceeds the single-sweep optimizer kernel (%d)", c->P, opt_max_params(c->opt_blocks)); return fail(MINPPO_ERR_UNSUPPORTED); }
  const int H = c->H, L = c->L, A = c->A;
  {
    int o = 0;
    c->po_w3a = o; o += H * A;
    c->po_b3a = o; o += A;
    o = (o + 3) / 4 * 4;
    c->po_w3c = o; o += H;
    c->po_b3c = o; o += 1;
    c->po_logstd = o; o += A;
    c->po_bh_a = o; o += H;
    c->po_bh_c = o; o += H;
    for (int net = 0; net < 2; ++net)
      for (int l = 0; l < 2; ++l) { c->po_db[net][l] = o; o += H; }
    c->po_loss = o; o += 2;
    c->head_stride = (o + 3) / 4 * 4;
  }
  const int EM = c->E * c->M;
#define ALLOC(ptr, n) if ((rc = dev_alloc(c, &(ptr), (n)))) return fail(rc)
  ALLOC(c->adv, static_cast<size_t>(c->Bl));
  ALLOC(c->tgt, static_cast<size_t>(c->Bl));
  ALLOC(c->stats, static_cast<size_t>(2 * EM));
  c->xchg = nullptr; c->peers_set = false; memset(&c->px, 0, sizeof(c->px)); memset(c->peer_ptr, 0, sizeof(c->peer_ptr));
  if (cfg->world_size > 1) {
    const int np = static_cast<int>((c->P + 2 + 3) / 4 * 4);
    const size_t floats = 2 * static_cast<size_t>(cfg->world_size) * np + static_cast<size_t>(cfg->world_size) * 256 + 2 * static_cast<size_t>(np);
    ALLOC(c->xchg, floats);
    fill_u32_kernel<<<296, 256>>>(reinterpret_cast<uint32_t*>(c->xchg), floats, 0x80000000u);
    ALLOC(c->xseq, 1);
    c->px.np = np; c->px.world = 0; c->px.rank = cfg->rank; c->px.seq = c->xseq;
  }
  ALLOC(c->gflat, static_cast<size_t>(c->P) + 4);
  ALLOC(c->block_ss, static_cast<size_t>(c->opt_blocks));
  ALLOC(c->head_part, static_cast<size_t>(c->tiles64) * c->head_stride);
  ALLOC(c->gnorms, static_cast<size_t>(EM));
  ALLOC(c->losses_scratch, 4);
  ALLOC(c->trace, static_cast<size_t>(2 * c->m_tiles) * FS_TRACE_SLOTS);
  ALLOC(c->trace2, static_cast<size_t>(c->sm_count) * 16);
  c->trace_on = getenv("MINPPO_TRACE") != nullptr;
  c->pdl = !(getenv("MINPPO_PDL") && atoi(getenv("MINPPO_PDL")) == 0);
  c->merged_opt = !(getenv("MINPPO_SPLIT_OPT") && atoi(getenv("MINPPO_SPLIT_OPT")) != 0);
  c->skip_mask = getenv("MINPPO_SKIP") ? atoi(getenv("MINPPO_SKIP")) : 0;
  c->persistent = getenv("MINPPO_PERSISTENT") && atoi(getenv("MINPPO_PERSISTENT")) != 0;
  c->steps_per_launch = getenv("MINPPO_STEPS_PER_LAUNCH") ? atoi(getenv("MINPPO_STEPS_PER_LAUNCH")) : 0;
  ALLOC(c->perms, static_cast<size_t>(c->E) * c->B);
  c->perm_tmp = nullptr;
  c->share_perm = cfg->world_size > 1 && !(getenv("MINPPO_SHARE_PERM") && atoi(getenv("MINPPO_SHARE_PERM")) == 0);
  if (c->share_perm) ALLOC(c->perm_tmp, static_cast<size_t>((c->E + cfg->world_size - 1) / cfg->world_size) * c->B);
  ALLOC(c->rowidx, static_cast<size_t>(EM) * c->cap);
  ALLOC(c->counts, static_cast<size_t>(EM));
  c->perm_ws_bytes = perm_workspace_bytes(c->E, c->B);
  { uint8_t* p; ALLOC(p, c->perm_ws_bytes); c->perm_ws = p; }
  ALLOC(c->obs_img, static_cast<size_t>(c->Bl) * c->Dp + 256);
  ALLOC(c->xg, static_cast<size_t>(c->M_pad) * c->Dp);
  if ((rc = make_tmap(&c->m_xg_k, c->xg, c->Dp, c->M_pad, c->Dp, 64, 128))) return fail(rc);
  if ((rc = make_tmap(&c->m_xg_mn, c->xg, c->Dp, c->M_pad, c->Dp, 64, 64))) return fail(rc);
  ALLOC(c->barrier, 1);
  ALLOC(c->err_flag, 1);
  for (int net = 0; net < 2; ++net) {
    NetBufs& nb = c->net[net];
    nb.act.assign(L + 1, nullptr); nb.dz.assign(L + 1, nullptr); nb.wn.assign(L, nullptr);
    nb.dw_part.assign(L, nullptr); nb.colsum.assign(L, nullptr); nb.dbias.assign(L, nullptr);
    ALLOC(nb.w2img, static_cast<size_t>(H) * FS_MAX_AP * 4);
    nb.m_act_k.resize(L + 1); nb.m_act_mn.resize(L + 1); nb.m_dz_k.resize(L + 1); nb.m_dz_mn.resize(L + 1);
    nb.m_wn_mn.resize(L); nb.m_wn.resize(2 * L); nb.m_dw.resize(L); nb.m_wn_h.resize(L);
    for (int l = 1; l <= L; ++l) {
      ALLOC(nb.act[l], static_cast<size_t>(c->M_pad) * H);
      ALLOC(nb.dz[l], static_cast<size_t>(c->M_pad) * H);
      if ((rc = make_tmap(&nb.m_act_k[l], nb.act[l], H, c->M_pad, H, 64, 128))) return fail(rc);
      if ((rc = make_tmap(&nb.m_act_mn[l], nb.act[l], H, c->M_pad, H, 64, 64))) return fail(rc);
      if ((rc = make_tmap(&nb.m_dz_k[l], nb.dz[l], H, c->M_pad, H, 64, 128))) return fail(rc);
      if ((rc = make_tmap(&nb.m_dz_mn[l], nb.dz[l], H, c->M_pad, H, 64, 64))) return fail(rc);
    }
    for (int l = 0; l < L; ++l) {
      const int kp = l == 0 ? c->Dp : H;
      const int in_l = l == 0 ? c->D : H;
      ALLOC(nb.wn[l], static_cast<size_t>(kp) * H);
      if ((rc = make_tmap(&nb.m_wn_mn[l], nb.wn[l], H, kp, H, 64, 64))) return fail(rc);
      if ((rc = make_tmap(&nb.m_wn_h[l], nb.wn[l], H, kp, H, 64, 32))) return fail(rc);
      if (l == 1 && (rc = make_tmap(&nb.m_w1k_h, nb.wn[l], H, H, H, 64, H / 2))) return fail(rc);
      if (l >= 1) {
        for (int j = 0; j < c->hsplit; ++j) {
          int n_off, n;
          col_group(H, c->hsplit, j, &n_off, &n);
          if ((rc = make_tmap(&nb.m_wn[2 * l + j], nb.wn[l], H, H, H, 64, n))) return fail(rc);
        }
        ALLOC(nb.colsum[l], static_cast<size_t>(c->m_tiles) * H);
      }
      ALLOC(nb.dw_part[l], static_cast<size_t>(c->S) * in_l * H);
      ALLOC(nb.dbias[l], static_cast<size_t>(c->S) * H);
      if ((rc = make_tmap_f32_3d(&nb.m_dw[l], nb.dw_part[l], H, in_l, c->S))) return fail(rc);
    }
  }
  c->pol_tiles = (c->Nl + 127) / 128;
  {
    const size_t prow = static_cast<size_t>(c->pol_tiles) * 128;
    ALLOC(c->pol_img, prow * c->Dp);
    if ((rc = make_tmap(&c->m_pol_img_k, c->pol_img, c->Dp, prow, c->Dp, 64, 128))) return fail(rc);
    for (int net = 0; net < 2; ++net)
      for (int l = 1; l <= L; ++l) {
        ALLOC(c->pol_act[net][l], prow * H);
        if ((rc = make_tmap(&c->m_pol_act_k[net][l], c->pol_act[net][l], H, prow, H, 64, 128))) return fail(rc);
      }
  }
#undef ALLOC
  if (cfg->world_size > 1) {
    NcclApi* api = nccl_api();
    if (!api) { set_error("libnccl.so.2 could not be loaded"); return fail(MINPPO_ERR_NCCL); }
    if (!nccl_unique_id_host) { set_error("world_size > 1 requires a NCCL unique id"); return fail(MINPPO_ERR_ARG); }
    ncclUniqueId id;
    memcpy(&id, nccl_unique_id_host, 128);
    ncclResult_t r = api->CommInitRank(&c->comm, cfg->world_size, id, cfg->rank);
    if (r != ncclSuccess) { set_error("ncclCommInitRank: %s", api->GetErrorString(r)); return fail(MINPPO_ERR_NCCL); }
    c->have_comm = true;
  }
  if (cudaStreamCreateWithFlags(&c->side_stream, cudaStreamNonBlocking) != cudaSuccess ||
      cudaEventCreateWithFlags(&c->ev_fork, cudaEventDisableTiming) != cudaSuccess ||
      cudaEventCreateWithFlags(&c->ev_join, cudaEventDisableTiming) != cudaSuccess) {
    set_error("side stream / event creation failed");
    return fail(MINPPO_ERR_CUDA);
  }
  if (cudaStreamCreateWithFlags(&c->cap_stream, cudaStreamNonBlocking) != cudaSuccess) {
    set_error("cudaStreamCreate failed");
    return fail(MINPPO_ERR_CUDA);
  }
  if (cudaDeviceSynchronize() != cudaSuccess) { set_error("context initialisation failed: %s", cudaGetErrorString(cudaGetLastError())); return fail(MINPPO_ERR_CUDA); }
  *out = c;
  return 0;
}

int minppo_update(minppo_ctx* c, float* params, float* mu, float* nu, int32_t* count, const float* obs,
                  const float* action, const float* value, const float* reward, const float* log_prob,
                  const uint8_t* done, const float* last_val, const uint32_t* key_in, uint32_t* key_out,
                  float* losses_out, int32_t use_graph, void* stream_v) {
  if (!c || !params || !mu || !nu || !count || !obs || !action || !value || !reward || !log_prob || !done ||
      !last_val || !key_in) {
    set_error("minppo_update: null pointer");
    return MINPPO_ERR_ARG;
  }
  cudaStream_t stream = static_cast<cudaStream_t>(stream_v);
  UpdatePtrs u;
  memset(&u, 0, sizeof(u));
  u.params = params; u.mu = mu; u.nu = nu; u.count = count; u.obs = obs; u.action = action; u.value = value;
  u.reward = reward; u.log_prob = log_prob; u.done = done; u.last_val = last_val; u.key_in = key_in;
  u.key_out = key_out; u.losses_out = losses_out;
  if (!use_graph) return enqueue_update(c, u, stream);
  const bool was_profiling = c->profiling;
  c->profiling = false;
  struct Restore { minppo_ctx* c; bool v; ~Restore() { c->profiling = v; } } restore{c, was_profiling};
  size_t hit = c->graphs.size();
  for (size_t i = 0; i < c->graphs.size(); ++i)
    if (c->graphs[i].ptrs == u) { hit = i; break; }
  if (hit == c->graphs.size()) {
    constexpr size_t kMaxGraphs = 4;
    if (c->graphs.size() >= kMaxGraphs) {
      cudaGraphExecDestroy(c->graphs.front().exec); cudaGraphDestroy(c->graphs.front().graph);
      c->graphs.erase(c->graphs.begin());
    }
    CK(cudaStreamBeginCapture(c->cap_stream, cudaStreamCaptureModeThreadLocal));
    int r = enqueue_update(c, u, c->cap_stream);
    cudaGraph_t g = nullptr;
    cudaError_t e = cudaStreamEndCapture(c->cap_stream, &g);
    if (r != 0) { if (g) cudaGraphDestroy(g); return r; }
    if (e != cudaSuccess) { set_error("graph capture failed: %s", cudaGetErrorString(e)); return MINPPO_ERR_CUDA; }
    cudaGraphExec_t ge = nullptr;
    if (cudaGraphInstantiate(&ge, g, 0) != cudaSuccess) { cudaGraphDestroy(g); set_error("cudaGraphInstantiate failed: %s", cudaGetErrorString(cudaGetLastError())); return MINPPO_ERR_CUDA; }
    c->graphs.push_back({g, ge, u, c->launches});
  } else if (hit + 1 != c->graphs.size()) {
    const minppo_ctx::CachedGraph cg = c->graphs[hit];
    c->graphs.erase(c->graphs.begin() + hit);
    c->graphs.push_back(cg);
  }
  c->launches = c->graphs.back().launches;
  CK(cudaGraphLaunch(c->graphs.back().exec, stream));
  return 0;
}

int minppo_policy_step(minppo_ctx* c, const float* params, const float* obs, const uint32_t* key_in, uint32_t* key_out,
                       float* action, float* log_prob, float* value, float* mean, int32_t flags, void* stream_v) {
  if (!c || !params || !obs) { set_error("minppo_policy_step: null pointer"); return MINPPO_ERR_ARG; }
  if (key_in && key_out == key_in) { set_error("minppo_policy_step: key_out must not alias key_in"); return MINPPO_ERR_ARG; }
  const bool actor = action || log_prob || mean;
  if (!actor && !value) { set_error("minppo_policy_step: no output requested"); return MINPPO_ERR_ARG; }
  cudaStream_t stream = static_cast<cudaStream_t>(stream_v);
  const int L = c->L, H = c->H;
  if (c->fused && !(getenv("MINPPO_POLICY_LAYERWISE") && atoi(getenv("MINPPO_POLICY_LAYERWISE")) != 0)) {
    if (!(flags & MINPPO_POLICY_WEIGHTS_CURRENT)) {
      UpdatePtrs u;
      memset(&u, 0, sizeof(u));
      u.params = const_cast<float*>(params);
      OptArgs o;
      fill_opt_args(c, u, &o);
      RET(weight_images_launch(o, stream));
    }
    PolicyParams pp;
    memset(&pp, 0, sizeof(pp));
    for (int net = 0; net < 2; ++net) {
      PolicyNet& g = pp.net[net];
      NetBufs& nb = c->net[net];
      g.tm_w0 = nb.m_wn_h[0]; g.tm_w1 = nb.m_wn_h[1];
      g.b0 = params + find_leaf(c, net, 0, 0).offset;
      g.b1 = params + find_leaf(c, net, 1, 0).offset;
      g.w2img = reinterpret_cast<const uint4*>(nb.w2img);
      g.b2 = params + find_leaf(c, net, 2, 0).offset;
      g.act = act_kind(c, net);
      g.aout = net == 0 ? c->A : 1;
    }
    pp.obs = obs; pp.log_std = params + c->leaves.back().offset;
    pp.key_in = actor ? key_in : nullptr; pp.key_out = actor ? key_out : nullptr;
    pp.action = action; pp.log_prob = log_prob; pp.value = value; pp.mean_out = mean;
    pp.n0 = c->n0; pp.n_total = static_cast<long long>(c->N) * c->A;
    pp.rows = c->Nl; pp.D = c->D; pp.Dp = c->Dp; pp.H = H; pp.A = c->A; pp.mode = c->cfg.prng_mode;
    pp.net_first = actor ? 0 : 1;
    const cudaError_t e = policy_fused_launch(pp, c->pol_tiles, stream, c->ap);
    if (e != cudaSuccess) { set_error("policy_fused launch failed: %s", cudaGetErrorString(e)); return MINPPO_ERR_CUDA; }
    return 0;
  }
  RET(obs_image_launch(obs, c->pol_img, c->Nl, c->D, c->Dp, stream));
  if (!(flags & MINPPO_POLICY_WEIGHTS_CURRENT)) {
    UpdatePtrs u;
    memset(&u, 0, sizeof(u));
    u.params = const_cast<float*>(params);
    OptArgs o;
    fill_opt_args(c, u, &o);
    RET(weight_images_launch(o, stream));
  }
  const int first = actor ? 0 : 1;
  for (int l = 0; l < L; ++l) {
    GemmParams p;
    memset(&p, 0, sizeof(p));
    int ng = 0;
    for (int i = first * c->hsplit; i < 2 * c->hsplit; ++i) {
      const int net = i / c->hsplit;
      GemmGroup& g = p.g[ng];
      g.cta_begin = ng * c->pol_tiles;
      ++ng;
      col_group(H, c->hsplit, i % c->hsplit, &g.n_off, &g.N);
      g.bmode = B_TMA_MN; g.tmB = c->net[net].m_wn_mn[l];
      g.amode = A_TMA_K;
      if (l == 0) { g.tmA = c->m_pol_img_k; g.kb_total = c->Dp / 64; }
      else { g.tmA = c->m_pol_act_k[net][l]; g.kb_total = H / 64; }
      g.out = c->pol_act[net][l + 1]; g.ldo = H;
      g.bias = params + find_leaf(c, net, l, 0).offset;
      g.act = act_kind(c, net);
      g.m_tiles = c->pol_tiles; g.splits = 1; g.m_store = c->pol_tiles * 128;
    }
    p.ngroups = ng;
    RET(launch_gemm<EPI_ACT>(p, ng * c->pol_tiles, stream));
  }
  PolicyHeadArgs a;
  memset(&a, 0, sizeof(a));
  a.h_a = actor ? c->pol_act[0][L] : nullptr;
  a.h_c = c->pol_act[1][L];
  a.params = params;
  a.off_w3a = static_cast<int>(find_leaf(c, 0, L, 1).offset); a.off_b3a = static_cast<int>(find_leaf(c, 0, L, 0).offset);
  a.off_w3c = static_cast<int>(find_leaf(c, 1, L, 1).offset); a.off_b3c = static_cast<int>(find_leaf(c, 1, L, 0).offset);
  a.off_logstd = static_cast<int>(c->leaves.back().offset);
  a.H = H; a.A = c->A; a.ldh = H; a.rows = c->Nl;
  a.n0 = c->n0; a.n_total = static_cast<long long>(c->N) * c->A;
  a.key_in = actor ? key_in : nullptr; a.key_out = actor ? key_out : nullptr; a.mode = c->cfg.prng_mode;
  a.action = action; a.log_prob = log_prob; a.value = value; a.mean_out = mean;
  return policy_head_launch(a, stream);
}

int minppo_ctx_ipc_handle(minppo_ctx* c, void* handle64_host) {
  if (!c || !handle64_host) { set_error("null argument"); return MINPPO_ERR_ARG; }
  if (!c->xchg) { set_error("minppo_ctx_ipc_handle: context has world_size == 1"); return MINPPO_ERR_ARG; }
  static_assert(sizeof(cudaIpcMemHandle_t) == 64, "cudaIpcMemHandle_t is 64 bytes");
  cudaIpcMemHandle_t h;
  CK(cudaIpcGetMemHandle(&h, c->xchg));
  memcpy(handle64_host, &h, 64);
  return 0;
}

int minppo_ctx_set_peers(minppo_ctx* c, const void* handles_host) {
  if (!c || !handles_host) { set_error("null argument"); return MINPPO_ERR_ARG; }
  if (!c->xchg) { set_error("minppo_ctx_set_peers: context has world_size == 1"); return MINPPO_ERR_ARG; }
  const int W = c->cfg.world_size;
  if (W > MINPPO_MAX_RANKS) { set_error("peer exchange supports up to %d ranks", MINPPO_MAX_RANKS); return MINPPO_ERR_UNSUPPORTED; }
  for (int r = 0; r < W; ++r) {
    if (r == c->cfg.rank) { c->px.base[r] = reinterpret_cast<char*>(c->xchg); continue; }
    cudaIpcMemHandle_t h;
    memcpy(&h, static_cast<const char*>(handles_host) + 64 * r, 64);
    void* ptr = nullptr;
    CK(cudaIpcOpenMemHandle(&ptr, h, cudaIpcMemLazyEnablePeerAccess));
    c->peer_ptr[r] = ptr;
    c->px.base[r] = static_cast<char*>(ptr);
  }
  c->px.world = W;
  c->px.two_phase = getenv("MINPPO_PX_TWO_PHASE") ? (atoi(getenv("MINPPO_PX_TWO_PHASE")) != 0) : (W >= 4);
  c->peers_set = true;
  drop_graphs(c);
  return 0;
}

int minppo_ctx_check(minppo_ctx* c, void* stream_v) {
  if (!c) return MINPPO_ERR_ARG;
  cudaStream_t stream = static_cast<cudaStream_t>(stream_v);
  CK(cudaStreamSynchronize(stream));
  int flag = 0;
  CK(cudaMemcpy(&flag, c->err_flag, sizeof(int), cudaMemcpyDeviceToHost));
  if (flag) { set_error("device-side error flag %d", flag); return flag; }
  const int EM = c->E * c->M;
  std::vector<int32_t> counts(EM);
  CK(cudaMemcpy(counts.data(), c->counts, EM * sizeof(int32_t), cudaMemcpyDeviceToHost));
  for (int s = 0; s < EM; ++s)
    if (counts[s] > c->cap) { set_error("minibatch %d: %d local rows exceed capacity %d", s, counts[s], c->cap); return MINPPO_ERR_WORKSPACE; }
  std::vector<float> gn(EM);
  CK(cudaMemcpy(gn.data(), c->gnorms, EM * sizeof(float), cudaMemcpyDeviceToHost));
  for (int s = 0; s < EM; ++s)
    if (!isfinite(gn[s])) { set_error("non-finite gradient norm at minibatch step %d", s); return MINPPO_ERR_NONFINITE; }
  return 0;
}

int64_t minppo_update_launch_count(const minppo_ctx* c) { return c ? c->launches : 0; }

int minppo_ctx_profile(minppo_ctx* c, int32_t enable) {
  if (!c) return MINPPO_ERR_ARG;
  c->profiling = enable != 0;
  c->prof_used = 0;
  return 0;
}

int minppo_ctx_profile_read(minppo_ctx* c, float* ms_per_class_host, int32_t* launches_per_class_host, int32_t nclasses) {
  if (!c || !ms_per_class_host || !launches_per_class_host) { set_error("null argument"); return MINPPO_ERR_ARG; }
  CK(cudaDeviceSynchronize());
  for (int i = 0; i < nclasses; ++i) { ms_per_class_host[i] = 0.f; launches_per_class_host[i] = 0; }
  for (size_t i = 0; i + 1 < c->prof_used; i += 2) {
    float ms = 0.f;
    CK(cudaEventElapsedTime(&ms, c->prof_events[i], c->prof_events[i + 1]));
    const int cls = c->prof_class[i / 2];
    if (cls < nclasses) { ms_per_class_host[cls] += ms; launches_per_class_host[cls] += 1; }
  }
  return 0;
}

int minppo_ctx_read(minppo_ctx* c, int32_t what, void* dst, size_t bytes, void* stream_v) {
  if (!c || !dst) { set_error("null argument"); return MINPPO_ERR_ARG; }
  const void* src = nullptr;
  size_t have = 0;
  const size_t EM = static_cast<size_t>(c->E) * c->M;
  switch (what) {
    case 0: src = c->adv; have = c->Bl * 4; break;
    case 1: src = c->tgt; have = c->Bl * 4; break;
    case 2: src = c->perms; have = static_cast<size_t>(c->E) * c->B * 4; break;
    case 3: src = c->gflat; have = (c->P + 4) * 4; break;
    case 4: src = c->gnorms; have = EM * 4; break;
    case 5: src = c->counts; have = EM * 4; break;
    case 6: src = c->stats; have = 2 * EM * 4; break;
    case 7: src = c->trace; have = static_cast<size_t>(2 * c->m_tiles) * FS_TRACE_SLOTS * 8; break;
    case 8: src = c->trace2; have = static_cast<size_t>(c->sm_count) * 16 * 8; break;
    default: set_error("minppo_ctx_read: unknown buffer %d", what); return MINPPO_ERR_ARG;
  }
  if (bytes > have) { set_error("minppo_ctx_read: %zu bytes requested, buffer has %zu", bytes, have); return MINPPO_ERR_ARG; }
  CK(cudaMemcpyAsync(dst, src, bytes, cudaMemcpyDeviceToDevice, static_cast<cudaStream_t>(stream_v)));
  return 0;
}

int minppo_debug_gemm(int32_t mode, const void* a_bf16, const void* b_bf16, const int32_t* rowidx, float* cmat,
                      int32_t M, int32_t N, int32_t K, int32_t lda, int32_t splits, void* stream_v) {
  if (!a_bf16 || !b_bf16 || !cmat || M % 128 || K % 64 || N % 64 || N > 256 || N <= 0 || splits < 1 || mode < 0 ||
      mode > 3 || ((mode >= 2) && !rowidx)) {
    set_error("minppo_debug_gemm: bad argument");
    return MINPPO_ERR_ARG;
  }
  RET(init_kernel_attrs());
  GemmParams p;
  memset(&p, 0, sizeof(p));
  p.ngroups = 1;
  GemmGroup& g = p.g[0];
  g.cta_begin = 0; g.N = N; g.m_tiles = M / 128; g.splits = splits; g.kb_total = K / 64; g.m_store = M;
  RET(make_tmap_f32_3d(&g.tmC, cmat, N, M, splits));
  switch (mode) {
    case 0:
      g.amode = A_TMA_K; g.bmode = B_TMA_K;
      RET(make_tmap(&g.tmA, a_bf16, K, M, lda ? lda : K, 64, 128));
      RET(make_tmap(&g.tmB, b_bf16, K, N, K, 64, N));
      break;
    case 1:
      g.amode = A_TMA_MN; g.bmode = B_TMA_MN;
      RET(make_tmap(&g.tmA, a_bf16, M, K, lda ? lda : M, 64, 64));
      RET(make_tmap(&g.tmB, b_bf16, N, K, N, 64, 64));
      break;
    case 2:
      g.amode = A_GATHER_K; g.bmode = B_TMA_K; g.rowidx = rowidx;
      g.gimage = reinterpret_cast<const __nv_bfloat16*>(a_bf16); g.ldg = lda;
      RET(make_tmap(&g.tmB, b_bf16, K, N, K, 64, N));
      break;
    case 3:
      g.amode = A_GATHER_MN; g.bmode = B_TMA_MN; g.rowidx = rowidx;
      g.gimage = reinterpret_cast<const __nv_bfloat16*>(a_bf16); g.ldg = lda;
      RET(make_tmap(&g.tmB, b_bf16, N, K, N, 64, 64));
      break;
  }
  return launch_gemm<EPI_PARTIAL>(p, g.m_tiles * splits, static_cast<cudaStream_t>(stream_v));
}

}
```

### minppo_b200/csrc/minppo_internal.h

```cpp
#pragma once

#include <cuda_bf16.h>
#include <cuda_runtime.h>
#include <stddef.h>
#include <stdint.h>

#include "../../include/minppo_b200.h"

namespace minppo {

enum : int { ACTK_TANH = 0, ACTK_RELU = 1, ACTK_TANH_FAST = 2 };

constexpr int MAX_HIDDEN = 512;

void gae_plan(int T, long long N, int sm_count, int* vec, int* chunks, int* seg_len);
int gae_launch(const float* reward, const float* value, const uint8_t* done, const float* last_val, float* adv,
               float* tgt, int T, long long N, float gamma, float gl, int sm_count, int force_chunks,
               cudaStream_t stream);

size_t perm_workspace_bytes(int epochs, long long B);
int perm_launch(const uint32_t* key_in_dev, uint32_t* key_out_dev, int mode, int epochs, long long B,
                int32_t* perm_out, void* ws, size_t ws_bytes, cudaStream_t stream, int epoch_first = 0,
                int epoch_step = 1, int key_epochs = -1);
int perm_launch_count(long long B);

int compact_rows_launch(const int32_t* perms, int32_t* rowidx, int32_t* counts, int E, int M, long long B, int mb,
                        int cap, int N, int n0, int Nl, int* err_flag, cudaStream_t stream);
int adv_stats_launch(const float* adv, const int32_t* rowidx, const int32_t* counts, float* stats, int EM, int cap,
                     int mb, int pass, cudaStream_t stream);

struct HeadLossArgs {
  const __nv_bfloat16* h_a;
  const __nv_bfloat16* h_c;
  __nv_bfloat16* dz_a;
  __nv_bfloat16* dz_c;
  const float* params;
  const int32_t* rowidx;
  const int32_t* count;
  const float* adv_sum;
  const float* adv_sq;
  const float* action;
  const float* v_old;
  const float* logp_old;
  const float* adv;
  const float* tgt;
  float* partials;
  int partial_stride;
  int po_w3a, po_b3a, po_w3c, po_b3c, po_logstd, po_bh_a, po_bh_c, po_loss;
  int off_w3a, off_b3a, off_w3c, off_b3c, off_logstd;
  int H, A, ldh, cap;
  int act_a, act_c;
  float inv_mb, clip_eps, vf_coef;
};
int head_loss_init();
int head_loss_launch(const HeadLossArgs& a, int tiles, cudaStream_t stream);

struct PolicyHeadArgs {
  const __nv_bfloat16* h_a;
  const __nv_bfloat16* h_c;
  const float* params;
  int off_w3a, off_b3a, off_w3c, off_b3c, off_logstd;
  int H, A, ldh;
  int rows;
  long long n0;
  long long n_total;
  const uint32_t* key_in;
  uint32_t* key_out;
  int mode;
  float* action;
  float* log_prob;
  float* value;
  float* mean_out;
};
int policy_head_launch(const PolicyHeadArgs& a, cudaStream_t stream);

struct OptLeaf {
  int offset;
  int cols;
  const float* grad_src;
  int src_offset;
  int nparts;
  int part_stride;
  float grad_bias;
  __nv_bfloat16* img_t;
  __nv_bfloat16* img_n;
  int ld_t, ld_n;
  uint8_t* img_w2;
  int late;
  int size;
  int ap;
};
struct OptArgs {
  OptLeaf leaf[MINPPO_MAX_LEAVES];
  int nleaves, P, A;
  int n_early;
  int do_reduce, do_apply;
  int keep_gflat;
  float* gflat;
  const float* loss_src;
  int loss_src_offset, loss_nparts, loss_part_stride;
  float* params; float* mu; float* nu;
  int32_t* count;
  float* block_ss;
  unsigned long long* barrier;
  int* err_flag;
  float* losses_out;
  float* gnorm_out;
  int off_logstd;
  int anneal, anneal_div, num_updates;
  float lr, max_norm, b1, b2, one_minus_b1, one_minus_b2, eps, eps_root;
  float inv_mb, vf_coef, ent_coef, entropy_const;
};
int opt_launch(const OptArgs& a, int blocks, cudaStream_t stream, bool pdl = false);
int opt_max_params(int blocks);
int weight_images_launch(const OptArgs& a, cudaStream_t stream);
int obs_image_launch(const float* obs, __nv_bfloat16* img, long long rows, int cols, int ld, cudaStream_t stream);

template <typename Kern, typename Arg>
inline cudaError_t launch_kernel(Kern kern, unsigned grid, unsigned block, size_t smem, cudaStream_t stream, bool pdl,
                                 const Arg& arg) {
  cudaLaunchConfig_t cfg = {};
  cfg.gridDim = dim3(grid, 1, 1);
  cfg.blockDim = dim3(block, 1, 1);
  cfg.dynamicSmemBytes = smem;
  cfg.stream = stream;
  cudaLaunchAttribute at[1];
  at[0].id = cudaLaunchAttributeProgrammaticStreamSerialization;
  at[0].val.programmaticStreamSerializationAllowed = 1;
  cfg.attrs = at;
  cfg.numAttrs = pdl ? 1 : 0;
  return cudaLaunchKernelEx(&cfg, kern, arg);
}

template <typename... KArgs, typename... Args>
inline cudaError_t launch_chain(void (*kern)(KArgs...), dim3 grid, dim3 block, size_t smem, cudaStream_t stream, Args... args) {
  cudaLaunchConfig_t cfg = {};
  cfg.gridDim = grid;
  cfg.blockDim = block;
  cfg.dynamicSmemBytes = smem;
  cfg.stream = stream;
  cudaLaunchAttribute at[1];
  at[0].id = cudaLaunchAttributeProgrammaticStreamSerialization;
  at[0].val.programmaticStreamSerializationAllowed = 1;
  cfg.attrs = at;
  cfg.numAttrs = 1;
  return cudaLaunchKernelEx(&cfg, kern, static_cast<KArgs>(args)...);
}

void set_error(const char* fmt, ...);

}
```

### minppo_b200/csrc/umma_gemm.cuh

```cuda
#pragma once

#include "common.cuh"

namespace minppo {

constexpr int GEMM_BM = 128;
constexpr int GEMM_BK = 64;
constexpr int GEMM_MAXN = 256;
constexpr int GEMM_STAGES = 4;
constexpr int GEMM_A_BYTES = GEMM_BM * GEMM_BK * 2;
constexpr int GEMM_B_BYTES = GEMM_MAXN * GEMM_BK * 2;
constexpr int GEMM_STAGE_BYTES = GEMM_A_BYTES + GEMM_B_BYTES;
constexpr int GEMM_THREADS = 192;
constexpr int GEMM_EPI_THREADS = 128;
constexpr int GEMM_ONES_BYTES = 16384;
constexpr int GEMM_SMEM_BYTES = GEMM_STAGES * GEMM_STAGE_BYTES + GEMM_ONES_BYTES + 1024  + 4 * GEMM_MAXN * 4  + 256;
constexpr int GEMM_MAX_GROUPS = 8;

enum : int { A_TMA_K = 0, A_GATHER_K = 1, A_TMA_MN = 2, A_GATHER_MN = 3 };
enum : int { B_TMA_K = 0, B_TMA_MN = 2 };
enum : int { EPI_ACT = 0, EPI_DACT = 1, EPI_PARTIAL = 2 };
enum : int { ACT_TANH = 0, ACT_RELU = 1, ACT_TANH_FAST = 2 };

struct alignas(64) GemmGroup {
  CUtensorMap tmA;
  CUtensorMap tmB;
  CUtensorMap tmC;
  const int32_t* rowidx;
  const __nv_bfloat16* gimage;
  void* out;
  const float* bias;
  const __nv_bfloat16* hprev;
  float* colsum;
  float* colsum_out;
  int ldg, ldo, ldh;
  int amode, bmode;
  int cta_begin;
  int act;
  int N;
  int m_tiles;
  int splits;
  int kb_total;
  int m_store;
  int n_off;
  int ldc;
  const int32_t* k_count;
};

static_assert(sizeof(GemmGroup) == 512, "GemmGroup grew: the kernel parameter blocks grow with it");

struct alignas(64) GemmParams {
  int ngroups;
  int grp_begin[GEMM_MAX_GROUPS];
  GemmGroup g[GEMM_MAX_GROUPS];
};
inline void gemm_finalize(GemmParams& p) {
  for (int i = 0; i < GEMM_MAX_GROUPS; ++i) p.grp_begin[i] = i < p.ngroups ? p.g[i].cta_begin : 0x7fffffff;
}

MINPPO_DEVINL void gather_line(uint32_t tile_base, int line, const __nv_bfloat16* src) {
  const uint32_t dst = tile_base + line * 128;
  const int sw = line & 7;
#pragma unroll
  for (int j = 0; j < 8; ++j) cp_async_16(dst + ((j ^ sw) << 4), reinterpret_cast<const char*>(src) + j * 16);
}

MINPPO_DEVINL float warp_colsum32(float (&v)[32]) {
  const uint32_t lane = lane_id();
#pragma unroll
  for (int half = 16; half >= 1; half >>= 1) {
    const bool upper = (lane & half) != 0;
#pragma unroll
    for (int i = 0; i < half; ++i) {
      float keep = upper ? v[i + half] : v[i];
      float send = upper ? v[i] : v[i + half];
      v[i] = keep + __shfl_xor_sync(0xffffffffu, send, half);
    }
  }
  return v[0];
}

struct GemmNoIdle { MINPPO_DEVINL void operator()() const {} };
constexpr uint32_t GEMM_NO_TMEM = 0xFFFFFFFFu;
template <int EPI, typename IdleFn = GemmNoIdle>
MINPPO_DEVINL void umma_gemm_body(const GemmParams& p, uint8_t* smem_raw, long long* trace = nullptr, IdleFn idle = IdleFn(),
                                  uint32_t ext_tmem = GEMM_NO_TMEM, const int32_t* step_rowidx = nullptr,
                                  const int32_t* step_kcount = nullptr) {
#define GEMM_STAMP(slot) do { if (trace) trace[(slot)] = clock64(); } while (0)
  const uint32_t raw = smem_u32(smem_raw);
  const uint32_t base = (raw + 1023u) & ~1023u;
  uint8_t* aligned = smem_raw + (base - raw);
  const uint32_t ones = base + GEMM_STAGES * GEMM_STAGE_BYTES;
  float* colsum_s = reinterpret_cast<float*>(aligned + GEMM_STAGES * GEMM_STAGE_BYTES + GEMM_ONES_BYTES);
  uint64_t* bars = reinterpret_cast<uint64_t*>(aligned + GEMM_STAGES * GEMM_STAGE_BYTES + GEMM_ONES_BYTES + 4 * GEMM_MAXN * 4);
  uint64_t* full_bar = bars;
  uint64_t* empty_bar = bars + GEMM_STAGES;
  uint64_t* tmem_full_bar = bars + 2 * GEMM_STAGES;
  uint32_t* tmem_slot = reinterpret_cast<uint32_t*>(bars + 2 * GEMM_STAGES + 1);
  uint64_t* chunk_bar = bars + 2 * GEMM_STAGES + 2;

  const int warp = threadIdx.x >> 5;
  int grp = 0;
#pragma unroll
  for (int i = 1; i < GEMM_MAX_GROUPS; ++i) grp += static_cast<int>(blockIdx.x) >= p.grp_begin[i] ? 1 : 0;
  const GemmGroup& G = p.g[grp];
  const int rem = static_cast<int>(blockIdx.x) - G.cta_begin;
  const int AMODE = G.amode, BMODE = G.bmode;
  const int m_tile = rem / G.splits;
  const int split = rem % G.splits;
  const int32_t* kcount = step_kcount ? step_kcount : G.k_count;
  const int kb_total = kcount ? min(G.kb_total, (max(*kcount, 0) + GEMM_BK - 1) / GEMM_BK) : G.kb_total;
  const int kb_per = (kb_total + G.splits - 1) / G.splits;
  const int kb0 = split * kb_per;
  const int kb1 = min(kb_total, kb0 + kb_per);
  const int nkb = max(0, kb1 - kb0);
  const int N = G.N;
  const bool kGather = (AMODE == A_GATHER_K || AMODE == A_GATHER_MN);
  const bool kTmaA = !kGather;
  const bool cs_even = (N % G.m_tiles) == 0 && ((N / G.m_tiles) % 64) == 0;
  const int cs_nc = cs_even ? N / G.m_tiles : (m_tile == 0 ? N : 0);
  const int cs_c0 = cs_even ? m_tile * cs_nc : 0;
  const bool kColsum = EPI == EPI_PARTIAL && G.colsum_out != nullptr && BMODE == B_TMA_MN && cs_nc > 0;
  constexpr uint32_t kTmemCols = EPI == EPI_PARTIAL ? 512 : 256;
  if (kColsum) {
    for (int i = threadIdx.x; i < GEMM_ONES_BYTES / 16; i += blockDim.x)
      sts128(ones + i * 16, make_uint4(0x3F803F80u, 0x3F803F80u, 0x3F803F80u, 0x3F803F80u));
    fence_proxy_async_smem();
  }

  if (threadIdx.x == 0) {
    GEMM_STAMP(13);
    if (kTmaA) tma_prefetch_desc(&G.tmA);
    tma_prefetch_desc(&G.tmB);
    if (EPI == EPI_PARTIAL) tma_prefetch_desc(&G.tmC);
    for (int s = 0; s < GEMM_STAGES; ++s) {
      mbar_init(&full_bar[s], 1 + (kGather ? GEMM_EPI_THREADS : 0));
      mbar_init(&empty_bar[s], 1);
    }
    mbar_init(tmem_full_bar, 1);
    for (int c = 0; c < GEMM_MAXN / 32; ++c) mbar_init(&chunk_bar[c], 4);
    fence_mbar_init();
    GEMM_STAMP(15);
  }
  if (warp == 1 && ext_tmem == GEMM_NO_TMEM) {
    tmem_alloc(tmem_slot, kTmemCols);
    tmem_relinquish();
  }
  tc_fence_before();
  __syncthreads();
  tc_fence_after();
  const uint32_t tmem_base = ext_tmem == GEMM_NO_TMEM ? *tmem_slot : ext_tmem;
  if (threadIdx.x == 64) GEMM_STAMP(6);

  const int nwarps = static_cast<int>(blockDim.x) >> 5;
  const int pq = warp & 3;
  const int first_helper = 6 + ((pq - 2) & 3);
  const int helpers_q = (EPI == EPI_PARTIAL && first_helper < nwarps) ? (nwarps - 1 - first_helper) / 4 + 1 : 0;
  const int drain_members = 1 + helpers_q;
  const int drain_idx = warp < 6 ? 0 : 1 + (warp - first_helper) / 4;

  if (warp == 0) {
    if (elect_one()) {
      griddep_wait();
      griddep_launch();
      if (ext_tmem != GEMM_NO_TMEM)
        fence_proxy_async_global();
      GEMM_STAMP(7);
      const uint32_t a_bytes = kTmaA ? GEMM_A_BYTES : 0;
      const uint32_t b_bytes = static_cast<uint32_t>(N) * GEMM_BK * 2;
      for (int i = 0; i < nkb; ++i) {
        const int s = i % GEMM_STAGES;
        const uint32_t ph = (i / GEMM_STAGES) & 1;
        mbar_wait(&empty_bar[s], ph ^ 1);
        const uint32_t sa = base + s * GEMM_STAGE_BYTES;
        const uint32_t sb = sa + GEMM_A_BYTES;
        mbar_arrive_expect_tx(&full_bar[s], a_bytes + b_bytes);
        const int kb = kb0 + i;
        if (AMODE == A_TMA_K) {
          tma_load_2d(sa, &G.tmA, &full_bar[s], kb * GEMM_BK, m_tile * GEMM_BM);
        } else if (AMODE == A_TMA_MN) {
          tma_load_2d(sa, &G.tmA, &full_bar[s], m_tile * GEMM_BM, kb * GEMM_BK);
          tma_load_2d(sa + 8192, &G.tmA, &full_bar[s], m_tile * GEMM_BM + 64, kb * GEMM_BK);
        }
        if (BMODE == B_TMA_K) {
          tma_load_2d(sb, &G.tmB, &full_bar[s], kb * GEMM_BK, G.n_off);
        } else {
          for (int c = 0; c < N / 64; ++c)
            tma_load_2d(sb + c * 8192, &G.tmB, &full_bar[s], G.n_off + c * 64, kb * GEMM_BK);
        }
      }
    }
  } else if (warp == 1) {
    if (elect_one()) {
      const uint32_t idesc = umma_idesc_bf16(GEMM_BM, static_cast<uint32_t>(N),
                                             (AMODE == A_TMA_MN || AMODE == A_GATHER_MN) ? 1u : 0u,
                                             (BMODE == B_TMA_MN) ? 1u : 0u);
      for (int i = 0; i < nkb; ++i) {
        const int s = i % GEMM_STAGES;
        const uint32_t ph = (i / GEMM_STAGES) & 1;
        mbar_wait(&full_bar[s], ph);
        tc_fence_after();
        if (i == 0) GEMM_STAMP(8);
        const uint32_t sa = base + s * GEMM_STAGE_BYTES;
        const uint32_t sb = sa + GEMM_A_BYTES;
#pragma unroll
        for (int j = 0; j < GEMM_BK / 16; ++j) {
          uint64_t da, db;
          if (AMODE == A_TMA_K || AMODE == A_GATHER_K) da = umma_smem_desc(sa + j * 32, 16, 1024);
          else da = umma_smem_desc(sa + j * 2048, 8192, 1024);
          if (BMODE == B_TMA_K) db = umma_smem_desc(sb + j * 32, 16, 1024);
          else db = umma_smem_desc(sb + j * 2048, 8192, 1024);
          umma_bf16(tmem_base, da, db, idesc, (i > 0 || j > 0) ? 1u : 0u);
          if (kColsum)
            umma_bf16(tmem_base + 256, umma_smem_desc(ones + j * 32, 16, 1024),
                      umma_smem_desc(sb + j * 2048 + (cs_c0 >> 6) * 8192, 8192, 1024),
                      umma_idesc_bf16(GEMM_BM, static_cast<uint32_t>(cs_nc), 0u, 1u), (i > 0 || j > 0) ? 1u : 0u);
        }
        umma_commit(&empty_bar[s]);
      }
      umma_commit(tmem_full_bar);
      GEMM_STAMP(9);
      if (EPI == EPI_PARTIAL) {
        for (int c = 0; c < N / 32; ++c) {
          mbar_wait(&chunk_bar[c], 0);
          if (c == 0) GEMM_STAMP(11);
          tma_store_3d(base + c * 16384, &G.tmC, G.n_off + c * 32, m_tile * GEMM_BM, split);
        }
        tma_store_commit();
        tma_store_wait_all0();
        fence_proxy_async_global();
        GEMM_STAMP(12);
      }
    }
  } else if (warp < GEMM_THREADS / 32) {
    const int et = threadIdx.x - 64;
    if (kGather) {
      const int32_t* ridx = step_rowidx ? step_rowidx : G.rowidx;
      constexpr int LAG = GEMM_STAGES - 1;
      const int c = et >> 6, kr = et & 63;
      const int row_k = (AMODE == A_GATHER_K) ? ridx[m_tile * GEMM_BM + et] : 0;
      int rows[8];
      for (int i = 0; i < nkb; ++i) {
        if ((i & 7) == 0 && AMODE == A_GATHER_MN) {
#pragma unroll
          for (int u = 0; u < 8; ++u) rows[u] = (i + u < nkb) ? ridx[(kb0 + i + u) * GEMM_BK + kr] : 0;
        }
        const int s = i % GEMM_STAGES;
        const uint32_t ph = (i / GEMM_STAGES) & 1;
        mbar_wait(&empty_bar[s], ph ^ 1);
        const uint32_t sa = base + s * GEMM_STAGE_BYTES;
        const int kb = kb0 + i;
        if (AMODE == A_GATHER_K) {
          gather_line(sa, et, G.gimage + static_cast<size_t>(row_k) * G.ldg + kb * GEMM_BK);
        } else {
          int row = rows[0];
#pragma unroll
          for (int u = 1; u < 8; ++u) row = ((i & 7) == u) ? rows[u] : row;
          gather_line(sa + c * 8192, kr, G.gimage + static_cast<size_t>(row) * G.ldg + m_tile * GEMM_BM + c * 64);
        }
        cp_async_commit();
        if (i >= LAG) {
          cp_async_wait<LAG>();
          fence_proxy_async_smem();
          mbar_arrive(&full_bar[(i - LAG) % GEMM_STAGES]);
        }
      }
      for (int j = max(0, nkb - LAG); j < nkb; ++j) {
        const int left = nkb - 1 - j;
        if (left >= 2) cp_async_wait<2>();
        else if (left == 1) cp_async_wait<1>();
        else cp_async_wait<0>();
        fence_proxy_async_smem();
        mbar_arrive(&full_bar[j % GEMM_STAGES]);
      }
    }

    const int q = warp & 3;
    const int row = m_tile * GEMM_BM + q * 32 + static_cast<int>(lane_id());
    if (nkb > 0) {
      mbar_wait(tmem_full_bar, 0);
      tc_fence_after();
    }
    if (et == 0) GEMM_STAMP(10);
    const uint32_t taddr = tmem_base + (static_cast<uint32_t>(q * 32) << 16);
    const int ldc = G.ldc ? G.ldc : N;
    for (int c0 = 32 * drain_idx; c0 < N; c0 += 32 * drain_members) {
      float v[32];
      if (nkb > 0) {
        tmem_ld_32x32(taddr + c0, v);
        tmem_ld_wait();
      } else {
#pragma unroll
        for (int j = 0; j < 32; ++j) v[j] = 0.f;
      }
      if (EPI == EPI_ACT) {
        const float* bp = G.bias + G.n_off + c0;
        uint32_t w[16];
#pragma unroll
        for (int j = 0; j < 8; ++j) {
          float x0 = v[4 * j] + __ldg(bp + 4 * j), x1 = v[4 * j + 1] + __ldg(bp + 4 * j + 1);
          float x2 = v[4 * j + 2] + __ldg(bp + 4 * j + 2), x3 = v[4 * j + 3] + __ldg(bp + 4 * j + 3);
          if (G.act == ACT_RELU) {
            x0 = fmaxf(x0, 0.f); x1 = fmaxf(x1, 0.f); x2 = fmaxf(x2, 0.f); x3 = fmaxf(x3, 0.f);
          } else if (G.act == ACT_TANH_FAST) {
            x0 = fast_tanh(x0); x1 = fast_tanh(x1); x2 = fast_tanh(x2); x3 = fast_tanh(x3);
          } else {
            x0 = exp_tanh(x0); x1 = exp_tanh(x1); x2 = exp_tanh(x2); x3 = exp_tanh(x3);
          }
          w[2 * j] = pack_bf16x2(x0, x1);
          w[2 * j + 1] = pack_bf16x2(x2, x3);
        }
        uint4* o = reinterpret_cast<uint4*>(reinterpret_cast<__nv_bfloat16*>(G.out) + static_cast<size_t>(row) * G.ldo + G.n_off + c0);
#pragma unroll
        for (int j = 0; j < 4; ++j) o[j] = make_uint4(w[4 * j], w[4 * j + 1], w[4 * j + 2], w[4 * j + 3]);
      } else if (EPI == EPI_DACT) {
        const uint4* h4 = reinterpret_cast<const uint4*>(G.hprev + static_cast<size_t>(row) * G.ldh + G.n_off + c0);
        uint32_t w[16];
#pragma unroll
        for (int j = 0; j < 4; ++j) {
          const uint4 hh = __ldg(h4 + j);
          const uint32_t hw[4] = {hh.x, hh.y, hh.z, hh.w};
#pragma unroll
          for (int t = 0; t < 4; ++t) {
            const float h0 = bf16_lo(hw[t]), h1 = bf16_hi(hw[t]);
            float d0, d1;
            if (G.act == ACT_RELU) { d0 = h0 > 0.f ? 1.f : 0.f; d1 = h1 > 0.f ? 1.f : 0.f; }
            else { d0 = 1.f - h0 * h0; d1 = 1.f - h1 * h1; }
            const int e = 8 * j + 2 * t;
            v[e] *= d0; v[e + 1] *= d1;
            w[4 * j + t] = pack_bf16x2(v[e], v[e + 1]);
            v[e] = bf16_lo(w[4 * j + t]); v[e + 1] = bf16_hi(w[4 * j + t]);
          }
        }
        uint4* o = reinterpret_cast<uint4*>(reinterpret_cast<__nv_bfloat16*>(G.out) + static_cast<size_t>(row) * G.ldo + G.n_off + c0);
#pragma unroll
        for (int j = 0; j < 4; ++j) o[j] = make_uint4(w[4 * j], w[4 * j + 1], w[4 * j + 2], w[4 * j + 3]);
        const float cs = warp_colsum32(v);
        colsum_s[q * GEMM_MAXN + c0 + lane_id()] = cs;
      } else {
        const int r = q * 32 + static_cast<int>(lane_id());
        const uint32_t dst = base + (c0 >> 5) * 16384 + r * 128;
#pragma unroll
        for (int j = 0; j < 8; ++j)
          sts128(dst + ((j ^ (r & 7)) << 4),
                 make_uint4(__float_as_uint(v[4 * j]), __float_as_uint(v[4 * j + 1]), __float_as_uint(v[4 * j + 2]),
                            __float_as_uint(v[4 * j + 3])));
        fence_proxy_async_smem();
        __syncwarp();
        if (lane_id() == 0) mbar_arrive(&chunk_bar[c0 >> 5]);
      }
    }
    if (kColsum) {
      for (int ch = q; ch < cs_nc / 32; ch += 4) {
        float v[32];
        if (nkb > 0) {
          tmem_ld_32x32(taddr + 256 + ch * 32, v);
          tmem_ld_wait();
        } else {
#pragma unroll
          for (int j = 0; j < 32; ++j) v[j] = 0.f;
        }
        float out = v[0];
#pragma unroll
        for (int j = 1; j < 32; ++j) out = (static_cast<int>(lane_id()) == j) ? v[j] : out;
        G.colsum_out[static_cast<size_t>(split) * ldc + G.n_off + cs_c0 + ch * 32 + lane_id()] = out;
      }
    }
    if (EPI == EPI_DACT) {
      asm volatile("bar.sync 1, 128;" ::: "memory");
      for (int c = et; c < N; c += GEMM_EPI_THREADS) {
        const float s = (colsum_s[c] + colsum_s[GEMM_MAXN + c]) + (colsum_s[2 * GEMM_MAXN + c] + colsum_s[3 * GEMM_MAXN + c]);
        G.colsum[static_cast<size_t>(m_tile) * ldc + G.n_off + c] = s;
      }
    }
  }

  else if (EPI == EPI_PARTIAL) {
    const int r = pq * 32 + static_cast<int>(lane_id());
    idle();
    if (nkb > 0) {
      mbar_wait(tmem_full_bar, 0);
      tc_fence_after();
    }
    const uint32_t taddr = tmem_base + (static_cast<uint32_t>(pq * 32) << 16);
    for (int c0 = 32 * drain_idx; c0 < N; c0 += 32 * drain_members) {
      float v[32];
      if (nkb > 0) {
        tmem_ld_32x32(taddr + c0, v);
        tmem_ld_wait();
      } else {
#pragma unroll
        for (int j = 0; j < 32; ++j) v[j] = 0.f;
      }
      const uint32_t dst = base + (c0 >> 5) * 16384 + r * 128;
#pragma unroll
      for (int j = 0; j < 8; ++j)
        sts128(dst + ((j ^ (r & 7)) << 4),
               make_uint4(__float_as_uint(v[4 * j]), __float_as_uint(v[4 * j + 1]), __float_as_uint(v[4 * j + 2]),
                          __float_as_uint(v[4 * j + 3])));
      fence_proxy_async_smem();
      __syncwarp();
      if (lane_id() == 0) mbar_arrive(&chunk_bar[c0 >> 5]);
    }
  }

  tc_fence_before();
  __syncthreads();
  if (warp == 1 && ext_tmem == GEMM_NO_TMEM) tmem_dealloc(tmem_base, kTmemCols);
}

template <int EPI>
__global__ void __launch_bounds__(GEMM_THREADS, 1) umma_gemm_kernel(const __grid_constant__ GemmParams p) {
  extern __shared__ uint8_t smem_raw[];
  umma_gemm_body<EPI>(p, smem_raw);
}

}
```

### minppo_b200/learner.py

```python
from __future__ import annotations

import ctypes as C
import dataclasses
import os
from typing import Any, NamedTuple, Optional

import numpy as np
import torch

from . import _lib
from .config import Config, to_c_config
from .params import leaf_paths, leaf_shapes, param_count


class Memory(NamedTuple):
    done: torch.Tensor
    action: torch.Tensor
    value: torch.Tensor
    reward: torch.Tensor
    log_prob: torch.Tensor
    obs: torch.Tensor
    info: Any = None


@dataclasses.dataclass
class TrainState:
    params: torch.Tensor
    mu: torch.Tensor
    nu: torch.Tensor
    step: torch.Tensor

    @staticmethod
    def create(flat_params: np.ndarray, device: torch.device) -> "TrainState":
        p = torch.as_tensor(np.ascontiguousarray(flat_params, np.float32)).to(device)
        return TrainState(p, torch.zeros_like(p), torch.zeros_like(p), torch.zeros(1, dtype=torch.int32, device=device))


def _ptr(t: Optional[torch.Tensor]) -> Optional[int]:
    return None if t is None else t.data_ptr()


def _stream_ptr(device: torch.device) -> int:
    return torch.cuda.current_stream(device).cuda_stream


def _as_u8(done: torch.Tensor) -> torch.Tensor:
    if done.dtype == torch.bool:
        return done.view(torch.uint8)
    if done.dtype != torch.uint8:
        raise TypeError(f"done must be bool or uint8, got {done.dtype}")
    return done


def _check(t: torch.Tensor, name: str, dtype: torch.dtype, shape, device: torch.device) -> torch.Tensor:
    if t.dtype != dtype:
        raise TypeError(f"{name}: expected {dtype}, got {t.dtype}")
    if tuple(t.shape) != tuple(shape):
        raise ValueError(f"{name}: expected shape {tuple(shape)}, got {tuple(t.shape)}")
    if t.device != device:
        raise ValueError(f"{name}: expected device {device}, got {t.device}")
    if not t.is_contiguous():
        raise ValueError(f"{name}: must be contiguous (time-major [T, N, ...])")
    return t


def calculate_gae(mem_batch: Memory, last_val: torch.Tensor, gamma: float, gae_lambda: float,
                  chunks: int = 0):
    lib = _lib.load()
    dev = mem_batch.reward.device
    if dev.type != "cuda":
        raise ValueError("calculate_gae needs CUDA tensors; there is no CPU path")
    T, N = mem_batch.reward.shape
    reward = _check(mem_batch.reward, "reward", torch.float32, (T, N), dev)
    value = _check(mem_batch.value, "value", torch.float32, (T, N), dev)
    done = _check(_as_u8(mem_batch.done), "done", torch.uint8, (T, N), dev)
    last_val = _check(last_val, "last_val", torch.float32, (N,), dev)
    adv = torch.empty_like(reward)
    tgt = torch.empty_like(reward)
    with torch.cuda.device(dev):
        _lib.check(lib.minppo_gae_chunked(_ptr(reward), _ptr(value), _ptr(done), _ptr(last_val), _ptr(adv), _ptr(tgt),
                                          T, N, gamma, gae_lambda, chunks, _stream_ptr(dev)))
    return adv, tgt


def permutations(rng: torch.Tensor, batch_size: int, epochs: int, prng_mode: int = _lib.PRNG_LEGACY):
    lib = _lib.load()
    dev = rng.device
    if dev.type != "cuda":
        raise ValueError("permutations needs CUDA tensors; there is no CPU path")
    if rng.numel() != 2 or rng.element_size() != 4:
        raise ValueError("rng must hold two 32-bit words")
    perms = torch.empty((epochs, batch_size), dtype=torch.int32, device=dev)
    rng_out = torch.empty_like(rng)
    ws_bytes = lib.minppo_permutation_workspace_size(epochs, batch_size)
    ws = torch.empty(ws_bytes, dtype=torch.uint8, device=dev)
    with torch.cuda.device(dev):
        _lib.check(lib.minppo_permutation(_ptr(rng), _ptr(rng_out), prng_mode, epochs, batch_size, _ptr(perms),
                                          _ptr(ws), ws_bytes, _stream_ptr(dev)))
    return rng_out, perms


def nccl_unique_id() -> bytes:
    buf = C.create_string_buffer(128)
    _lib.check(_lib.load().minppo_nccl_unique_id(buf))
    return buf.raw


class Learner:

    def __init__(self, config: Config, obs_dim: int, act_dim: int, device: Optional[torch.device] = None,
                 world_size: int = 1, rank: int = 0, nccl_id: Optional[bytes] = None):
        self.lib = _lib.load()
        if not torch.cuda.is_available():
            raise RuntimeError("minppo_b200.Learner needs a CUDA (sm_100a) device; there is no CPU fallback")
        self.device = torch.device(device if device is not None else f"cuda:{torch.cuda.current_device()}")
        self.config = config
        self.obs_dim, self.act_dim = obs_dim, act_dim
        self.world_size, self.rank = world_size, rank
        self.cconf = to_c_config(config, obs_dim, act_dim, world_size, rank)
        t = config.training
        self.T, self.N = t.num_steps, t.num_envs
        self.Nl = self.N // world_size
        self.E, self.M = t.update_epochs, t.num_minibatches
        self.P = param_count(obs_dim, act_dim, config.model.hidden_size, config.model.num_layers)
        batch = self.T * self.N
        if (batch // self.M) * self.M != batch:
            raise ValueError("`batch_size` must be equal to `num_steps * num_envs`")
        handle = C.c_void_p()
        idbuf = C.create_string_buffer(nccl_id, 128) if nccl_id is not None else None
        with torch.cuda.device(self.device):
            _lib.check(self.lib.minppo_ctx_create(C.byref(self.cconf), idbuf, C.byref(handle)))
        self._h = handle
        self.use_graph = bool(config.learner.use_graph)
        self._key_in = torch.zeros(2, dtype=torch.int32, device=self.device)
        self._key_out = torch.zeros(2, dtype=torch.int32, device=self.device)
        self._losses = torch.zeros((self.E, self.M, 4), dtype=torch.float32, device=self.device)
        self.peer_exchange = False
        if world_size > 1 and os.environ.get("MINPPO_NCCL_ALLREDUCE", "0") != "1":
            self._connect_peers()

    def _connect_peers(self) -> None:
        import torch.distributed as dist

        if not (dist.is_available() and dist.is_initialized()) or dist.get_world_size() != self.world_size:
            return
        buf = C.create_string_buffer(64)
        with torch.cuda.device(self.device):
            _lib.check(self.lib.minppo_ctx_ipc_handle(self._h, buf))
            handles = [None] * self.world_size
            dist.all_gather_object(handles, buf.raw)
            table = C.create_string_buffer(b"".join(handles), 64 * self.world_size)
            _lib.check(self.lib.minppo_ctx_set_peers(self._h, table))
        dist.barrier()
        self.peer_exchange = True

    def close(self) -> None:
        if getattr(self, "_h", None):
            self.lib.minppo_ctx_destroy(self._h)
            self._h = None

    def __del__(self):
        try:
            self.close()
        except Exception:
            pass

    def param_layout(self):
        n = C.c_int32()
        offs = (C.c_int64 * _lib.MAX_LEAVES)()
        rows = (C.c_int64 * _lib.MAX_LEAVES)()
        cols = (C.c_int64 * _lib.MAX_LEAVES)()
        P = self.lib.minppo_param_layout(C.byref(self.cconf), C.byref(n), offs, rows, cols)
        paths = leaf_paths(self.config.model.num_layers)
        return P, [(paths[i], offs[i], rows[i], cols[i]) for i in range(n.value)]

    def update(self, train_state: TrainState, mem_batch: Memory, last_val: torch.Tensor, rng: torch.Tensor,
               losses: Optional[torch.Tensor] = None, rng_out: Optional[torch.Tensor] = None):
        dev = self.device
        T, Nl, D, A = self.T, self.Nl, self.obs_dim, self.act_dim
        obs = _check(mem_batch.obs, "obs", torch.float32, (T, Nl, D), dev)
        action = _check(mem_batch.action, "action", torch.float32, (T, Nl, A), dev)
        value = _check(mem_batch.value, "value", torch.float32, (T, Nl), dev)
        reward = _check(mem_batch.reward, "reward", torch.float32, (T, Nl), dev)
        log_prob = _check(mem_batch.log_prob, "log_prob", torch.float32, (T, Nl), dev)
        done = _check(_as_u8(mem_batch.done), "done", torch.uint8, (T, Nl), dev)
        last_val = _check(last_val, "last_val", torch.float32, (Nl,), dev)
        _check(train_state.params, "params", torch.float32, (self.P,), dev)
        _check(train_state.mu, "mu", torch.float32, (self.P,), dev)
        _check(train_state.nu, "nu", torch.float32, (self.P,), dev)
        _check(train_state.step, "step", torch.int32, (1,), dev)
        if rng.numel() != 2 or rng.element_size() != 4 or rng.device != dev:
            raise ValueError("rng must hold two 32-bit words on the learner's device")
        if losses is None:
            losses = self._losses
        else:
            _check(losses, "losses", torch.float32, (self.E, self.M, 4), dev)
        if rng_out is None:
            rng_out = self._key_out.view(rng.dtype)
        with torch.cuda.device(dev):
            if rng.data_ptr() != self._key_in.data_ptr():
                self._key_in.copy_(rng.reshape(2).view(torch.int32), non_blocking=True)
            _lib.check(self.lib.minppo_update(
                self._h, _ptr(train_state.params), _ptr(train_state.mu), _ptr(train_state.nu), _ptr(train_state.step),
                _ptr(obs), _ptr(action), _ptr(value), _ptr(reward), _ptr(log_prob), _ptr(done), _ptr(last_val),
                _ptr(self._key_in), _ptr(rng_out), _ptr(losses), int(self.use_graph), _stream_ptr(dev)))
        return train_state, rng_out, losses

    def policy_step(self, params: torch.Tensor, last_obs: torch.Tensor, rng: Optional[torch.Tensor],
                    weights_current: bool = False, want_mean: bool = False):
        dev = self.device
        obs = _check(last_obs, "last_obs", torch.float32, (self.Nl, self.obs_dim), dev)
        _check(params, "params", torch.float32, (self.P,), dev)
        if rng is not None and (rng.numel() != 2 or rng.element_size() != 4 or rng.device != dev):
            raise ValueError("rng must hold two 32-bit words on the learner's device")
        action = torch.empty((self.Nl, self.act_dim), dtype=torch.float32, device=dev)
        log_prob = torch.empty((self.Nl,), dtype=torch.float32, device=dev)
        value = torch.empty((self.Nl,), dtype=torch.float32, device=dev)
        mean = torch.empty_like(action) if want_mean else None
        rng_out = torch.empty_like(rng) if rng is not None else None
        with torch.cuda.device(dev):
            _lib.check(self.lib.minppo_policy_step(
                self._h, _ptr(params), _ptr(obs), _ptr(rng), _ptr(rng_out), _ptr(action), _ptr(log_prob), _ptr(value),
                _ptr(mean), _lib.POLICY_WEIGHTS_CURRENT if weights_current else 0, _stream_ptr(dev)))
        return action, log_prob, value, rng_out, mean

    def bootstrap_value(self, params: torch.Tensor, last_obs: torch.Tensor, weights_current: bool = False) -> torch.Tensor:
        dev = self.device
        obs = _check(last_obs, "last_obs", torch.float32, (self.Nl, self.obs_dim), dev)
        _check(params, "params", torch.float32, (self.P,), dev)
        value = torch.empty((self.Nl,), dtype=torch.float32, device=dev)
        with torch.cuda.device(dev):
            _lib.check(self.lib.minppo_policy_step(
                self._h, _ptr(params), _ptr(obs), None, None, None, None, _ptr(value), None,
                _lib.POLICY_WEIGHTS_CURRENT if weights_current else 0, _stream_ptr(dev)))
        return value

    def check(self) -> None:
        with torch.cuda.device(self.device):
            _lib.check(self.lib.minppo_ctx_check(self._h, _stream_ptr(self.device)))

    def launches_per_update(self) -> int:
        return int(self.lib.minppo_update_launch_count(self._h))

    _WHAT = {"advantages": 0, "targets": 1, "perms": 2, "grad": 3, "grad_norms": 4, "counts": 5, "adv_stats": 6}

    def read(self, what: str) -> torch.Tensor:
        EM, B, Bl = self.E * self.M, self.T * self.N, self.T * self.Nl
        spec = {
            "advantages": ((self.T, self.Nl), torch.float32), "targets": ((self.T, self.Nl), torch.float32),
            "perms": ((self.E, B), torch.int32), "grad": ((self.P + 4,), torch.float32),
            "grad_norms": ((EM,), torch.float32), "counts": ((EM,), torch.int32),
            "adv_stats": ((2, EM), torch.float32),
        }[what]
        out = torch.empty(spec[0], dtype=spec[1], device=self.device)
        with torch.cuda.device(self.device):
            _lib.check(self.lib.minppo_ctx_read(self._h, self._WHAT[what], _ptr(out), out.numel() * out.element_size(),
                                                _stream_ptr(self.device)))
        return out

    def update_host(self, host: "HostBatch") -> np.ndarray:
        host.to_device(self.device)
        ts = TrainState(host.d["params"], host.d["mu"], host.d["nu"], host.d["step"])
        mem = Memory(host.d["done"], host.d["action"], host.d["value"], host.d["reward"], host.d["log_prob"],
                     host.d["obs"])
        self.update(ts, mem, host.d["last_val"], host.d["rng"], host.d["losses"], host.d["rng_out"])
        host.to_host()
        torch.cuda.current_stream(self.device).synchronize()
        return host.h["losses"].numpy()


class HostBatch:
    IN = ("obs", "action", "value", "reward", "log_prob", "done", "last_val", "rng", "params", "mu", "nu", "step")
    OUT = ("params", "mu", "nu", "step", "rng_out", "losses")

    def __init__(self, learner: Learner):
        T, Nl, D, A, P = learner.T, learner.Nl, learner.obs_dim, learner.act_dim, learner.P
        f32, i32, u8 = torch.float32, torch.int32, torch.uint8
        spec = {
            "obs": ((T, Nl, D), f32), "action": ((T, Nl, A), f32), "value": ((T, Nl), f32), "reward": ((T, Nl), f32),
            "log_prob": ((T, Nl), f32), "done": ((T, Nl), u8), "last_val": ((Nl,), f32), "rng": ((2,), i32),
            "params": ((P,), f32), "mu": ((P,), f32), "nu": ((P,), f32), "step": ((1,), i32),
            "rng_out": ((2,), i32), "losses": ((learner.E, learner.M, 4), f32),
        }
        self.h = {k: torch.zeros(s, dtype=dt).pin_memory() for k, (s, dt) in spec.items()}
        self.d = {k: torch.empty(s, dtype=dt, device=learner.device) for k, (s, dt) in spec.items()}

    def h2d_bytes(self) -> int:
        return sum(self.h[k].numel() * self.h[k].element_size() for k in self.IN)

    def d2h_bytes(self) -> int:
        return sum(self.h[k].numel() * self.h[k].element_size() for k in self.OUT)

    def to_device(self, device) -> None:
        for k in self.IN:
            self.d[k].copy_(self.h[k], non_blocking=True)

    def to_host(self) -> None:
        for k in self.OUT:
            self.h[k].copy_(self.d[k], non_blocking=True)


class HostPipeline:

    DEPTH = 2

    def __init__(self, learner: Learner, train_state: TrainState, rng: torch.Tensor):
        self.lrn = learner
        self.ts = train_state
        dev = learner.device
        T, Nl, D, A, P = learner.T, learner.Nl, learner.obs_dim, learner.act_dim, learner.P
        f32, u8 = torch.float32, torch.uint8
        self.spec = {"obs": ((T, Nl, D), f32), "action": ((T, Nl, A), f32), "value": ((T, Nl), f32), "reward": ((T, Nl), f32),
                     "log_prob": ((T, Nl), f32), "done": ((T, Nl), u8), "last_val": ((Nl,), f32)}
        self.dev_in = [{k: torch.empty(s, dtype=dt, device=dev) for k, (s, dt) in self.spec.items()} for _ in range(self.DEPTH)]
        self.dev_losses = [torch.empty((learner.E, learner.M, 4), dtype=f32, device=dev) for _ in range(self.DEPTH)]
        self.host_out = [{"losses": torch.empty((learner.E, learner.M, 4), dtype=f32).pin_memory(),
                          "params": torch.empty((P,), dtype=f32).pin_memory(),
                          "rng": torch.empty((2,), dtype=torch.int32).pin_memory()} for _ in range(self.DEPTH)]
        self.rng = [rng.reshape(2).view(torch.int32).clone(), torch.empty(2, dtype=torch.int32, device=dev)]
        self.copy_stream = torch.cuda.Stream(device=dev)
        self.ev_copied = [torch.cuda.Event() for _ in range(self.DEPTH)]
        self.ev_done = [torch.cuda.Event() for _ in range(self.DEPTH)]
        self.ev_free = [None] * self.DEPTH
        self.n_submitted = 0
        self.n_returned = 0

    def h2d_bytes(self) -> int:
        return sum(int(np.prod(s)) * torch.empty((), dtype=dt).element_size() for s, dt in self.spec.values())

    def d2h_bytes(self) -> int:
        return sum(t.numel() * t.element_size() for t in self.host_out[0].values())

    def submit(self, traj: dict) -> None:
        if self.n_submitted - self.n_returned >= self.DEPTH:
            raise RuntimeError("HostPipeline: call result() before submitting a third update")
        k = self.n_submitted % self.DEPTH
        dev = self.lrn.device
        compute = torch.cuda.current_stream(dev)
        with torch.cuda.stream(self.copy_stream):
            if self.ev_free[k] is not None:
                self.copy_stream.wait_event(self.ev_free[k])
            for name in self.spec:
                src = traj[name]
                if name == "done" and src.dtype == torch.bool:
                    src = src.view(torch.uint8)
                self.dev_in[k][name].copy_(src, non_blocking=True)
            self.ev_copied[k].record(self.copy_stream)
        compute.wait_event(self.ev_copied[k])
        d = self.dev_in[k]
        mem = Memory(d["done"], d["action"], d["value"], d["reward"], d["log_prob"], d["obs"])
        i = self.n_submitted
        self.lrn.update(self.ts, mem, d["last_val"], self.rng[i % 2], self.dev_losses[k], self.rng[(i + 1) % 2])
        ev = torch.cuda.Event()
        ev.record(compute)
        self.ev_free[k] = ev
        h = self.host_out[k]
        h["losses"].copy_(self.dev_losses[k], non_blocking=True)
        h["params"].copy_(self.ts.params, non_blocking=True)
        h["rng"].copy_(self.rng[(i + 1) % 2], non_blocking=True)
        self.ev_done[k].record(compute)
        self.n_submitted += 1

    def result(self):
        if self.n_returned >= self.n_submitted:
            raise RuntimeError("HostPipeline: nothing outstanding")
        k = self.n_returned % self.DEPTH
        self.ev_done[k].synchronize()
        self.n_returned += 1
        return self.host_out[k]["losses"].numpy(), self.host_out[k]["params"].numpy()
```

Before: 50.10 million.

## Run weight-gradient GEMMs as 2-CTA cluster pairs with cta_group::2 UMMA

```diff
diff --git a/minppo_b200/csrc/common.cuh b/minppo_b200/csrc/common.cuh
--- a/minppo_b200/csrc/common.cuh
+++ b/minppo_b200/csrc/common.cuh
@@ -132,6 +132,27 @@
       : "memory");
 }
 
+MINPPO_DEVINL void tma_load_2d_pair(uint32_t smem_dst, const CUtensorMap* m, uint32_t bar_cluster, int c0, int c1) {
+  asm volatile(
+      "cp.async.bulk.tensor.2d.cta_group::2.shared::cluster.global.mbarrier::complete_tx::bytes"
+      " [%0], [%1, {%3, %4}], [%2];"
+      ::"r"(smem_dst), "l"(reinterpret_cast<uint64_t>(m)), "r"(bar_cluster), "r"(c0), "r"(c1)
+      : "memory");
+}
+
+MINPPO_DEVINL uint32_t cluster_ctarank() {
+  uint32_t r;
+  asm volatile("mov.u32 %0, %%cluster_ctarank;" : "=r"(r));
+  return r;
+}
+MINPPO_DEVINL uint32_t mapa_shared(uint32_t smem_addr, uint32_t rank) {
+  uint32_t d;
+  asm volatile("mapa.shared::cluster.u32 %0, %1, %2;" : "=r"(d) : "r"(smem_addr), "r"(rank));
+  return d;
+}
+MINPPO_DEVINL void cluster_arrive() { asm volatile("barrier.cluster.arrive.release.aligned;" ::: "memory"); }
+MINPPO_DEVINL void cluster_wait() { asm volatile("barrier.cluster.wait.acquire.aligned;" ::: "memory"); }
+
 MINPPO_DEVINL void tma_store_2d(uint32_t smem_src, const CUtensorMap* m, int c0, int c1) {
   asm volatile("cp.async.bulk.tensor.2d.global.shared::cta.bulk_group [%0, {%2, %3}], [%1];" ::"l"(
                    reinterpret_cast<uint64_t>(m)),
@@ -187,6 +208,30 @@
 }
 MINPPO_DEVINL void umma_commit(uint64_t* bar) {
   asm volatile("tcgen05.commit.cta_group::1.mbarrier::arrive::one.shared::cluster.b64 [%0];" ::"r"(smem_u32(bar))
+               : "memory");
+}
+
+MINPPO_DEVINL void tmem_alloc2(uint32_t* smem_dst, uint32_t ncols) {
+  asm volatile("tcgen05.alloc.cta_group::2.sync.aligned.shared::cta.b32 [%0], %1;" ::"r"(smem_u32(smem_dst)), "r"(ncols)
+               : "memory");
+}
+MINPPO_DEVINL void tmem_relinquish2() {
+  asm volatile("tcgen05.relinquish_alloc_permit.cta_group::2.sync.aligned;" ::: "memory");
+}
+MINPPO_DEVINL void tmem_dealloc2(uint32_t taddr, uint32_t ncols) {
+  asm volatile("tcgen05.dealloc.cta_group::2.sync.aligned.b32 %0, %1;" ::"r"(taddr), "r"(ncols) : "memory");
+}
+MINPPO_DEVINL void umma_bf16_pair(uint32_t tmem_d, uint64_t desc_a, uint64_t desc_b, uint32_t idesc, uint32_t accumulate) {
+  asm volatile(
+      "{\n\t.reg .pred p;\n\t"
+      "setp.ne.b32 p, %4, 0;\n\t"
+      "tcgen05.mma.cta_group::2.kind::f16 [%0], %1, %2, %3, p;\n\t}\n"
+      ::"r"(tmem_d), "l"(desc_a), "l"(desc_b), "r"(idesc), "r"(accumulate)
+      : "memory");
+}
+MINPPO_DEVINL void umma_commit_pair(uint64_t* bar, uint16_t cta_mask) {
+  asm volatile("tcgen05.commit.cta_group::2.mbarrier::arrive::one.shared::cluster.multicast::cluster.b64 [%0], %1;"
+               ::"r"(smem_u32(bar)), "h"(cta_mask)
                : "memory");
 }
 
diff --git a/minppo_b200/csrc/dwopt.cuh b/minppo_b200/csrc/dwopt.cuh
--- a/minppo_b200/csrc/dwopt.cuh
+++ b/minppo_b200/csrc/dwopt.cuh
@@ -90,8 +90,8 @@
   return s;
 }
 
-template <int MAXU>
-MINPPO_DEVINL void dwopt_body(const DwOptParams& p, int step, uint8_t* smem_raw, uint32_t ext_tmem, bool build_tab = true) {
+template <int MAXU, bool PAIR = false>
+MINPPO_DEVINL uint32_t dwopt_body(const DwOptParams& p, int step, uint8_t* smem_raw, uint32_t ext_tmem, bool build_tab = true) {
   __shared__ float scratch[32];
   __shared__ float s_bcast[4];
   __shared__ LeafTab T;
@@ -135,6 +135,7 @@
     }
   };
 
+  uint32_t tmem = GEMM_NO_TMEM;
   if (gemm_cta) {
     auto idle_work = [&]() {
       if (build_tab) leaf_tab_build(T, a, t - GEMM_THREADS, NT - GEMM_THREADS);
@@ -150,7 +151,7 @@
         }
       }
     };
-    umma_gemm_body<EPI_PARTIAL>(p.gemm, smem_raw, p.trace ? p.trace + static_cast<size_t>(b) * 16 : nullptr, idle_work, ext_tmem,
+    tmem = umma_gemm_body<EPI_PARTIAL, PAIR>(p.gemm, smem_raw, p.trace ? p.trace + static_cast<size_t>(b) * 16 : nullptr, idle_work, ext_tmem,
                                 p.ridx_base + static_cast<size_t>(step) * p.cap, row_count);
   } else {
     scalars();
@@ -204,7 +205,7 @@
   } else {
     ss += reduce_leaves<true>(a, T, gtid, GT_);
   }
-  if (!a.do_apply) return;
+  if (!a.do_apply) return tmem;
 
   if (px_on) {
     const PeerXchg& X = p.px;
@@ -426,20 +427,43 @@
       if (gnorm_out) *gnorm_out = sc.gnorm;
     }
   }
-}
-
-template <int MAXU>
+  return tmem;
+}
+
+template <int MAXU, bool PAIR>
 __global__ void __launch_bounds__(DWOPT_THREADS, 1) dwopt_kernel(const __grid_constant__ DwOptParams p) {
   extern __shared__ uint8_t smem_raw[];
-  dwopt_body<MAXU>(p, p.step, smem_raw, GEMM_NO_TMEM);
+  const uint32_t tmem = dwopt_body<MAXU, PAIR>(p, p.step, smem_raw, GEMM_NO_TMEM);
+  if (PAIR && tmem != GEMM_NO_TMEM) gemm_pair_release(tmem);
 }
 
 inline long long dwopt_fast_capacity(int grid, int maxu) { return 4LL * grid * DWOPT_THREADS * maxu; }
 
-inline cudaError_t dwopt_launch(const DwOptParams& p, int grid, cudaStream_t stream, bool pdl, int maxu) {
-  if (maxu <= 1) return launch_kernel(dwopt_kernel<1>, grid, DWOPT_THREADS, GEMM_SMEM_BYTES, stream, pdl, p);
-  if (maxu == 2) return launch_kernel(dwopt_kernel<2>, grid, DWOPT_THREADS, GEMM_SMEM_BYTES, stream, pdl, p);
-  return launch_kernel(dwopt_kernel<4>, grid, DWOPT_THREADS, GEMM_SMEM_BYTES, stream, pdl, p);
-}
-
-}
+inline cudaError_t dwopt_launch(const DwOptParams& p, int grid, cudaStream_t stream, bool pdl, int maxu, bool pairs) {
+  const int cluster = pairs ? 2 : 1;
+  if (pairs) {
+    if (maxu <= 1) return launch_kernel(dwopt_kernel<1, true>, grid, DWOPT_THREADS, GEMM_SMEM_BYTES, stream, pdl, p, cluster);
+    if (maxu == 2) return launch_kernel(dwopt_kernel<2, true>, grid, DWOPT_THREADS, GEMM_SMEM_BYTES, stream, pdl, p, cluster);
+    return launch_kernel(dwopt_kernel<4, true>, grid, DWOPT_THREADS, GEMM_SMEM_BYTES, stream, pdl, p, cluster);
+  }
+  if (maxu <= 1) return launch_kernel(dwopt_kernel<1, false>, grid, DWOPT_THREADS, GEMM_SMEM_BYTES, stream, pdl, p);
+  if (maxu == 2) return launch_kernel(dwopt_kernel<2, false>, grid, DWOPT_THREADS, GEMM_SMEM_BYTES, stream, pdl, p);
+  return launch_kernel(dwopt_kernel<4, false>, grid, DWOPT_THREADS, GEMM_SMEM_BYTES, stream, pdl, p);
+}
+
+inline int dwopt_max_pair_clusters() {
+  cudaLaunchConfig_t cfg = {};
+  cfg.gridDim = dim3(2, 1, 1);
+  cfg.blockDim = dim3(DWOPT_THREADS, 1, 1);
+  cfg.dynamicSmemBytes = GEMM_SMEM_BYTES;
+  cudaLaunchAttribute at[1];
+  at[0].id = cudaLaunchAttributeClusterDimension;
+  at[0].val.clusterDim.x = 2; at[0].val.clusterDim.y = 1; at[0].val.clusterDim.z = 1;
+  cfg.attrs = at;
+  cfg.numAttrs = 1;
+  int n = 0;
+  if (cudaOccupancyMaxActiveClusters(&n, dwopt_kernel<1, true>, &cfg) != cudaSuccess) { cudaGetLastError(); return 0; }
+  return n;
+}
+
+}
diff --git a/minppo_b200/csrc/learner.cu b/minppo_b200/csrc/learner.cu
--- a/minppo_b200/csrc/learner.cu
+++ b/minppo_b200/csrc/learner.cu
@@ -217,6 +217,9 @@
   int dw_nsplit;
   int hsplit;
   int maxu;
+  bool dw_pairs;
+  int dw_grid;
+  int32_t* dw_info;
   bool fused;
   int head_parts;
   std::vector<LeafInfo> leaves;
@@ -334,9 +337,12 @@
   if (head_loss_init()) { set_error("head_loss_init failed"); return MINPPO_ERR_CUDA; }
   CK(cudaFuncSetAttribute(fused_step_kernel<16>, cudaFuncAttributeMaxDynamicSharedMemorySize, FsLayout<16>::BYTES));
   CK(cudaFuncSetAttribute(fused_step_kernel<32>, cudaFuncAttributeMaxDynamicSharedMemorySize, FsLayout<32>::BYTES));
-  CK(cudaFuncSetAttribute(dwopt_kernel<1>, cudaFuncAttributeMaxDynamicSharedMemorySize, GEMM_SMEM_BYTES));
-  CK(cudaFuncSetAttribute(dwopt_kernel<2>, cudaFuncAttributeMaxDynamicSharedMemorySize, GEMM_SMEM_BYTES));
-  CK(cudaFuncSetAttribute(dwopt_kernel<4>, cudaFuncAttributeMaxDynamicSharedMemorySize, GEMM_SMEM_BYTES));
+  CK(cudaFuncSetAttribute(dwopt_kernel<1, false>, cudaFuncAttributeMaxDynamicSharedMemorySize, GEMM_SMEM_BYTES));
+  CK(cudaFuncSetAttribute(dwopt_kernel<2, false>, cudaFuncAttributeMaxDynamicSharedMemorySize, GEMM_SMEM_BYTES));
+  CK(cudaFuncSetAttribute(dwopt_kernel<4, false>, cudaFuncAttributeMaxDynamicSharedMemorySize, GEMM_SMEM_BYTES));
+  CK(cudaFuncSetAttribute(dwopt_kernel<1, true>, cudaFuncAttributeMaxDynamicSharedMemorySize, GEMM_SMEM_BYTES));
+  CK(cudaFuncSetAttribute(dwopt_kernel<2, true>, cudaFuncAttributeMaxDynamicSharedMemorySize, GEMM_SMEM_BYTES));
+  CK(cudaFuncSetAttribute(dwopt_kernel<4, true>, cudaFuncAttributeMaxDynamicSharedMemorySize, GEMM_SMEM_BYTES));
   CK(steps_init_attrs());
   CK(policy_fused_init_attrs());
   return 0;
@@ -447,7 +453,12 @@
   p.trace = c->trace_on ? c->trace : nullptr;
 }
 
-static int fill_dwopt_params(minppo_ctx* c, const UpdatePtrs& u, DwOptParams* dpp) {
+static int dw_tile_ctas(int in_pad, bool pairs) {
+  const int t = (in_pad + 127) / 128;
+  return pairs ? (t + 1) / 2 * 2 : t;
+}
+
+static int fill_dwopt_params(minppo_ctx* c, const UpdatePtrs& u, DwOptParams* dpp, bool pairs) {
   DwOptParams& dp = *dpp;
   memset(&dp, 0, sizeof(dp));
   const int L = c->L, H = c->H;
@@ -472,7 +483,7 @@
       col_group(H, c->dw_nsplit, nh, &g.n_off, &g.N);
       g.ldc = H;
       g.m_tiles = (in_pad + 127) / 128; g.splits = c->S; g.m_store = in_l;
-      cta += g.m_tiles * g.splits;
+      cta += dw_tile_ctas(in_pad, pairs) * g.splits;
       }
     }
   }
@@ -580,19 +591,21 @@
   }
   }
   DwOptParams dp;
-  const int cta = fill_dwopt_params(c, u, &dp);
+  const bool try_merged = c->merged_opt && c->skip_mask == 0;
+  int cta = fill_dwopt_params(c, u, &dp, try_merged && c->dw_pairs);
+  const bool merged = try_merged && cta <= c->dw_grid;
+  if (!merged && try_merged && c->dw_pairs) cta = fill_dwopt_params(c, u, &dp, false);
   dp.step = s;
   GemmParams& p = dp.gemm;
   OptArgs& o = dp.opt;
   const bool sharded = c->cfg.world_size > 1;
-  const bool merged = c->merged_opt && c->skip_mask == 0 && cta <= c->sm_count;
   if (merged) {
-    const bool px_on = sharded && c->peers_set && c->P <= dwopt_fast_capacity(c->sm_count, c->maxu);
+    const bool px_on = sharded && c->peers_set && c->P <= dwopt_fast_capacity(c->dw_grid, c->maxu);
     if (px_on) { dp.px = c->px; dp.px.ablate = getenv("MINPPO_PX_ABLATE") ? atoi(getenv("MINPPO_PX_ABLATE")) : 0; }
     o.do_reduce = 1; o.do_apply = (sharded && !px_on) ? 0 : 1;
     {
       PROF(PC_DW_GEMM);
-      const cudaError_t e = dwopt_launch(dp, c->sm_count, stream, pdl, c->maxu);
+      const cudaError_t e = dwopt_launch(dp, c->dw_grid, stream, pdl, c->maxu, c->dw_pairs);
       if (e != cudaSuccess) { set_error("dwopt launch failed: %s", cudaGetErrorString(e)); return MINPPO_ERR_CUDA; }
       c->launches++;
     }
@@ -708,7 +721,7 @@
     StepsParams sp;
     memset(&sp, 0, sizeof(sp));
     fill_fused_params(c, u, &sp.fs);
-    const int cta = fill_dwopt_params(c, u, &sp.dw);
+    const int cta = fill_dwopt_params(c, u, &sp.dw, false);
     const bool sharded = cfg.world_size > 1;
     const bool px_on = sharded && c->peers_set && c->P <= dwopt_fast_capacity(c->sm_count, c->maxu);
     if (cta <= c->sm_count && (!sharded || px_on)) {
@@ -865,14 +878,29 @@
   c->store_x = c->fused;
   c->head_parts = c->fused ? c->m_tiles : c->tiles64;
   c->P = build_layout(*cfg, &c->leaves);
-  c->maxu = c->P <= dwopt_fast_capacity(c->sm_count, 1) ? 1 : (c->P <= dwopt_fast_capacity(c->sm_count, 2) ? 2 : 4);
+  c->merged_opt = !(getenv("MINPPO_SPLIT_OPT") && atoi(getenv("MINPPO_SPLIT_OPT")) != 0);
+  c->skip_mask = getenv("MINPPO_SKIP") ? atoi(getenv("MINPPO_SKIP")) : 0;
+  c->persistent = getenv("MINPPO_PERSISTENT") && atoi(getenv("MINPPO_PERSISTENT")) != 0;
   {
     c->dw_nsplit = c->H > GEMM_MAXN ? 2
                  : (c->fused && c->store_x && c->H % 128 == 0 && 2 * 2 * c->L <= GEMM_MAX_GROUPS &&
                     !(getenv("MINPPO_DW_NSPLIT") && atoi(getenv("MINPPO_DW_NSPLIT")) == 1)) ? 2 : 1;
+    bool pairs = c->fused && c->store_x && c->merged_opt && c->skip_mask == 0 && !c->persistent &&
+                 !(getenv("MINPPO_DW_PAIRS") && atoi(getenv("MINPPO_DW_PAIRS")) == 0);
+    for (int j = 0; j < c->dw_nsplit; ++j) {
+      int n_off, n;
+      col_group(c->H, c->dw_nsplit, j, &n_off, &n);
+      if (n % 128) pairs = false;
+    }
+    const int clusters = pairs ? dwopt_max_pair_clusters() : 0;
+    if (clusters < 1) pairs = false;
+    for (;; pairs = false) {
+    c->dw_pairs = pairs;
+    c->dw_grid = pairs ? 2 * std::min(clusters, c->sm_count / 2) : c->sm_count;
+    c->maxu = c->P <= dwopt_fast_capacity(c->dw_grid, 1) ? 1 : (c->P <= dwopt_fast_capacity(c->dw_grid, 2) ? 2 : 4);
     int per_split = 0;
-    for (int l = 0; l < c->L; ++l) per_split += 2 * c->dw_nsplit * (((l == 0 ? c->Dp : c->H) + 127) / 128);
-    const int gemm_budget = c->sm_count > 48 ? c->sm_count - 16 : c->sm_count;
+    for (int l = 0; l < c->L; ++l) per_split += 2 * c->dw_nsplit * dw_tile_ctas(l == 0 ? c->Dp : c->H, pairs);
+    const int gemm_budget = c->dw_grid > 48 ? c->dw_grid - 16 : c->dw_grid;
     int S = cfg->dw_splits > 0 ? cfg->dw_splits : (gemm_budget / (per_split > 0 ? per_split : 1));
     if (getenv("MINPPO_DW_SPLITS")) S = atoi(getenv("MINPPO_DW_SPLITS"));
     int kb_total = c->M_pad / 64;
@@ -887,6 +915,8 @@
     if (S < 1) S = 1;
     while (S > 1 && ((kb_total + S - 1) / S) * (S - 1) >= kb_total) --S;
     c->S = S;
+    if (!pairs || (S * per_split <= c->dw_grid && c->P <= dwopt_fast_capacity(c->dw_grid, 4))) break;
+    }
   }
   c->opt_blocks = c->sm_count;
   if (c->P > opt_max_params(c->opt_blocks)) { set_error("parameter count %lld exceeds the single-sweep optimizer kernel (%d)", c->P, opt_max_params(c->opt_blocks)); return fail(MINPPO_ERR_UNSUPPORTED); }
@@ -927,11 +957,13 @@
   ALLOC(c->losses_scratch, 4);
   ALLOC(c->trace, static_cast<size_t>(2 * c->m_tiles) * FS_TRACE_SLOTS);
   ALLOC(c->trace2, static_cast<size_t>(c->sm_count) * 16);
+  ALLOC(c->dw_info, 4);
+  {
+    const int32_t info[4] = {c->dw_pairs ? 1 : 0, c->dw_grid, c->S, c->dw_nsplit};
+    if (cudaMemcpy(c->dw_info, info, sizeof(info), cudaMemcpyHostToDevice) != cudaSuccess) { set_error("dw_info upload failed"); return fail(MINPPO_ERR_CUDA); }
+  }
   c->trace_on = getenv("MINPPO_TRACE") != nullptr;
   c->pdl = !(getenv("MINPPO_PDL") && atoi(getenv("MINPPO_PDL")) == 0);
-  c->merged_opt = !(getenv("MINPPO_SPLIT_OPT") && atoi(getenv("MINPPO_SPLIT_OPT")) != 0);
-  c->skip_mask = getenv("MINPPO_SKIP") ? atoi(getenv("MINPPO_SKIP")) : 0;
-  c->persistent = getenv("MINPPO_PERSISTENT") && atoi(getenv("MINPPO_PERSISTENT")) != 0;
   c->steps_per_launch = getenv("MINPPO_STEPS_PER_LAUNCH") ? atoi(getenv("MINPPO_STEPS_PER_LAUNCH")) : 0;
   ALLOC(c->perms, static_cast<size_t>(c->E) * c->B);
   c->perm_tmp = nullptr;
@@ -1003,6 +1035,16 @@
     ncclResult_t r = api->CommInitRank(&c->comm, cfg->world_size, id, cfg->rank);
     if (r != ncclSuccess) { set_error("ncclCommInitRank: %s", api->GetErrorString(r)); return fail(MINPPO_ERR_NCCL); }
     c->have_comm = true;
+    float g2[2] = {static_cast<float>(c->dw_grid), -static_cast<float>(c->dw_grid)};
+    if (cudaMemcpy(c->gflat, g2, sizeof(g2), cudaMemcpyHostToDevice) != cudaSuccess) { set_error("dwopt grid upload failed"); return fail(MINPPO_ERR_CUDA); }
+    r = api->AllReduce(c->gflat, c->gflat, 2, ncclFloat, ncclMax, c->comm, nullptr);
+    if (r != ncclSuccess) { set_error("ncclAllReduce (dwopt grid): %s", api->GetErrorString(r)); return fail(MINPPO_ERR_NCCL); }
+    if (cudaMemcpy(g2, c->gflat, sizeof(g2), cudaMemcpyDeviceToHost) != cudaSuccess) { set_error("dwopt grid read-back failed"); return fail(MINPPO_ERR_CUDA); }
+    if (g2[0] != -g2[1]) {
+      set_error("ranks disagree on the dwopt grid (%d .. %d CTAs; this rank %d): set MINPPO_DW_PAIRS=0 on every rank",
+                static_cast<int>(-g2[1]), static_cast<int>(g2[0]), c->dw_grid);
+      return fail(MINPPO_ERR_UNSUPPORTED);
+    }
   }
   if (cudaStreamCreateWithFlags(&c->side_stream, cudaStreamNonBlocking) != cudaSuccess ||
       cudaEventCreateWithFlags(&c->ev_fork, cudaEventDisableTiming) != cudaSuccess ||
@@ -1240,6 +1282,7 @@
     case 6: src = c->stats; have = 2 * EM * 4; break;
     case 7: src = c->trace; have = static_cast<size_t>(2 * c->m_tiles) * FS_TRACE_SLOTS * 8; break;
     case 8: src = c->trace2; have = static_cast<size_t>(c->sm_count) * 16 * 8; break;
+    case 9: src = c->dw_info; have = 4 * 4; break;
     default: set_error("minppo_ctx_read: unknown buffer %d", what); return MINPPO_ERR_ARG;
   }
   if (bytes > have) { set_error("minppo_ctx_read: %zu bytes requested, buffer has %zu", bytes, have); return MINPPO_ERR_ARG; }
diff --git a/minppo_b200/csrc/minppo_internal.h b/minppo_b200/csrc/minppo_internal.h
--- a/minppo_b200/csrc/minppo_internal.h
+++ b/minppo_b200/csrc/minppo_internal.h
@@ -118,17 +118,26 @@
 
 template <typename Kern, typename Arg>
 inline cudaError_t launch_kernel(Kern kern, unsigned grid, unsigned block, size_t smem, cudaStream_t stream, bool pdl,
-                                 const Arg& arg) {
+                                 const Arg& arg, int cluster = 1) {
   cudaLaunchConfig_t cfg = {};
   cfg.gridDim = dim3(grid, 1, 1);
   cfg.blockDim = dim3(block, 1, 1);
   cfg.dynamicSmemBytes = smem;
   cfg.stream = stream;
-  cudaLaunchAttribute at[1];
-  at[0].id = cudaLaunchAttributeProgrammaticStreamSerialization;
-  at[0].val.programmaticStreamSerializationAllowed = 1;
+  cudaLaunchAttribute at[2];
+  int n = 0;
+  if (pdl) {
+    at[n].id = cudaLaunchAttributeProgrammaticStreamSerialization;
+    at[n].val.programmaticStreamSerializationAllowed = 1;
+    ++n;
+  }
+  if (cluster > 1) {
+    at[n].id = cudaLaunchAttributeClusterDimension;
+    at[n].val.clusterDim.x = static_cast<unsigned>(cluster); at[n].val.clusterDim.y = 1; at[n].val.clusterDim.z = 1;
+    ++n;
+  }
   cfg.attrs = at;
-  cfg.numAttrs = pdl ? 1 : 0;
+  cfg.numAttrs = n;
   return cudaLaunchKernelEx(&cfg, kern, arg);
 }
 
diff --git a/minppo_b200/csrc/umma_gemm.cuh b/minppo_b200/csrc/umma_gemm.cuh
--- a/minppo_b200/csrc/umma_gemm.cuh
+++ b/minppo_b200/csrc/umma_gemm.cuh
@@ -14,6 +14,10 @@
 constexpr int GEMM_THREADS = 192;
 constexpr int GEMM_EPI_THREADS = 128;
 constexpr int GEMM_ONES_BYTES = 16384;
+constexpr int GEMM_PAIR_STAGES = 6;
+constexpr int GEMM_PAIR_STAGE_BYTES = GEMM_A_BYTES + GEMM_B_BYTES / 2;
+static_assert(GEMM_PAIR_STAGES * GEMM_PAIR_STAGE_BYTES <= GEMM_STAGES * GEMM_STAGE_BYTES, "pair ring exceeds the ring region");
+static_assert((2 * GEMM_PAIR_STAGES + 2 + 8) * 8 <= 256, "pair-mode mbarriers exceed their 256-byte region");
 constexpr int GEMM_SMEM_BYTES = GEMM_STAGES * GEMM_STAGE_BYTES + GEMM_ONES_BYTES + 1024  + 4 * GEMM_MAXN * 4  + 256;
 constexpr int GEMM_MAX_GROUPS = 8;
 
@@ -82,22 +86,26 @@
 
 struct GemmNoIdle { MINPPO_DEVINL void operator()() const {} };
 constexpr uint32_t GEMM_NO_TMEM = 0xFFFFFFFFu;
-template <int EPI, typename IdleFn = GemmNoIdle>
-MINPPO_DEVINL void umma_gemm_body(const GemmParams& p, uint8_t* smem_raw, long long* trace = nullptr, IdleFn idle = IdleFn(),
+template <int EPI, bool PAIR = false, typename IdleFn = GemmNoIdle>
+MINPPO_DEVINL uint32_t umma_gemm_body(const GemmParams& p, uint8_t* smem_raw, long long* trace = nullptr, IdleFn idle = IdleFn(),
                                   uint32_t ext_tmem = GEMM_NO_TMEM, const int32_t* step_rowidx = nullptr,
                                   const int32_t* step_kcount = nullptr) {
 #define GEMM_STAMP(slot) do { if (trace) trace[(slot)] = clock64(); } while (0)
+  static_assert(!PAIR || EPI == EPI_PARTIAL, "pair mode is the split-K dW GEMM only");
+  constexpr int kStages = PAIR ? GEMM_PAIR_STAGES : GEMM_STAGES;
+  constexpr int kStageBytes = PAIR ? GEMM_PAIR_STAGE_BYTES : GEMM_STAGE_BYTES;
+  constexpr int kRing = GEMM_STAGES * GEMM_STAGE_BYTES;
   const uint32_t raw = smem_u32(smem_raw);
   const uint32_t base = (raw + 1023u) & ~1023u;
   uint8_t* aligned = smem_raw + (base - raw);
-  const uint32_t ones = base + GEMM_STAGES * GEMM_STAGE_BYTES;
-  float* colsum_s = reinterpret_cast<float*>(aligned + GEMM_STAGES * GEMM_STAGE_BYTES + GEMM_ONES_BYTES);
-  uint64_t* bars = reinterpret_cast<uint64_t*>(aligned + GEMM_STAGES * GEMM_STAGE_BYTES + GEMM_ONES_BYTES + 4 * GEMM_MAXN * 4);
+  const uint32_t ones = base + kRing;
+  float* colsum_s = reinterpret_cast<float*>(aligned + kRing + GEMM_ONES_BYTES);
+  uint64_t* bars = reinterpret_cast<uint64_t*>(aligned + kRing + GEMM_ONES_BYTES + 4 * GEMM_MAXN * 4);
   uint64_t* full_bar = bars;
-  uint64_t* empty_bar = bars + GEMM_STAGES;
-  uint64_t* tmem_full_bar = bars + 2 * GEMM_STAGES;
-  uint32_t* tmem_slot = reinterpret_cast<uint32_t*>(bars + 2 * GEMM_STAGES + 1);
-  uint64_t* chunk_bar = bars + 2 * GEMM_STAGES + 2;
+  uint64_t* empty_bar = bars + kStages;
+  uint64_t* tmem_full_bar = bars + 2 * kStages;
+  uint32_t* tmem_slot = reinterpret_cast<uint32_t*>(bars + 2 * kStages + 1);
+  uint64_t* chunk_bar = bars + 2 * kStages + 2;
 
   const int warp = threadIdx.x >> 5;
   int grp = 0;
@@ -106,8 +114,10 @@
   const GemmGroup& G = p.g[grp];
   const int rem = static_cast<int>(blockIdx.x) - G.cta_begin;
   const int AMODE = G.amode, BMODE = G.bmode;
-  const int m_tile = rem / G.splits;
-  const int split = rem % G.splits;
+  const int m_tile = PAIR ? 2 * ((rem >> 1) / G.splits) + (rem & 1) : rem / G.splits;
+  const int split = PAIR ? (rem >> 1) % G.splits : rem % G.splits;
+  const uint32_t pair_rank = PAIR ? cluster_ctarank() : 0u;
+  const bool mma_cta = pair_rank == 0;
   const int32_t* kcount = step_kcount ? step_kcount : G.k_count;
   const int kb_total = kcount ? min(G.kb_total, (max(*kcount, 0) + GEMM_BK - 1) / GEMM_BK) : G.kb_total;
   const int kb_per = (kb_total + G.splits - 1) / G.splits;
@@ -115,12 +125,12 @@
   const int kb1 = min(kb_total, kb0 + kb_per);
   const int nkb = max(0, kb1 - kb0);
   const int N = G.N;
-  const bool kGather = (AMODE == A_GATHER_K || AMODE == A_GATHER_MN);
+  const bool kGather = !PAIR && (AMODE == A_GATHER_K || AMODE == A_GATHER_MN);
   const bool kTmaA = !kGather;
   const bool cs_even = (N % G.m_tiles) == 0 && ((N / G.m_tiles) % 64) == 0;
   const int cs_nc = cs_even ? N / G.m_tiles : (m_tile == 0 ? N : 0);
   const int cs_c0 = cs_even ? m_tile * cs_nc : 0;
-  const bool kColsum = EPI == EPI_PARTIAL && G.colsum_out != nullptr && BMODE == B_TMA_MN && cs_nc > 0;
+  const bool kColsum = !PAIR && EPI == EPI_PARTIAL && G.colsum_out != nullptr && BMODE == B_TMA_MN && cs_nc > 0;
   constexpr uint32_t kTmemCols = EPI == EPI_PARTIAL ? 512 : 256;
   if (kColsum) {
     for (int i = threadIdx.x; i < GEMM_ONES_BYTES / 16; i += blockDim.x)
@@ -133,7 +143,7 @@
     if (kTmaA) tma_prefetch_desc(&G.tmA);
     tma_prefetch_desc(&G.tmB);
     if (EPI == EPI_PARTIAL) tma_prefetch_desc(&G.tmC);
-    for (int s = 0; s < GEMM_STAGES; ++s) {
+    for (int s = 0; s < kStages; ++s) {
       mbar_init(&full_bar[s], 1 + (kGather ? GEMM_EPI_THREADS : 0));
       mbar_init(&empty_bar[s], 1);
     }
@@ -142,12 +152,14 @@
     fence_mbar_init();
     GEMM_STAMP(15);
   }
+  if (PAIR) cluster_arrive();
   if (warp == 1 && ext_tmem == GEMM_NO_TMEM) {
-    tmem_alloc(tmem_slot, kTmemCols);
-    tmem_relinquish();
+    if (PAIR) { tmem_alloc2(tmem_slot, kTmemCols); tmem_relinquish2(); }
+    else { tmem_alloc(tmem_slot, kTmemCols); tmem_relinquish(); }
   }
   tc_fence_before();
   __syncthreads();
+  if (PAIR) cluster_wait();
   tc_fence_after();
   const uint32_t tmem_base = ext_tmem == GEMM_NO_TMEM ? *tmem_slot : ext_tmem;
   if (threadIdx.x == 64) GEMM_STAMP(6);
@@ -167,15 +179,24 @@
         fence_proxy_async_global();
       GEMM_STAMP(7);
       const uint32_t a_bytes = kTmaA ? GEMM_A_BYTES : 0;
-      const uint32_t b_bytes = static_cast<uint32_t>(N) * GEMM_BK * 2;
+      const uint32_t b_bytes = static_cast<uint32_t>(PAIR ? N / 2 : N) * GEMM_BK * 2;
       for (int i = 0; i < nkb; ++i) {
-        const int s = i % GEMM_STAGES;
-        const uint32_t ph = (i / GEMM_STAGES) & 1;
+        const int s = i % kStages;
+        const uint32_t ph = (i / kStages) & 1;
         mbar_wait(&empty_bar[s], ph ^ 1);
-        const uint32_t sa = base + s * GEMM_STAGE_BYTES;
+        const uint32_t sa = base + s * kStageBytes;
         const uint32_t sb = sa + GEMM_A_BYTES;
+        const int kb = kb0 + i;
+        if (PAIR) {
+          if (mma_cta) mbar_arrive_expect_tx(&full_bar[s], 2 * (a_bytes + b_bytes));
+          const uint32_t fb = mapa_shared(smem_u32(&full_bar[s]), 0);
+          tma_load_2d_pair(sa, &G.tmA, fb, m_tile * GEMM_BM, kb * GEMM_BK);
+          tma_load_2d_pair(sa + 8192, &G.tmA, fb, m_tile * GEMM_BM + 64, kb * GEMM_BK);
+          for (int c = 0; c < N / 128; ++c)
+            tma_load_2d_pair(sb + c * 8192, &G.tmB, fb, G.n_off + static_cast<int>(pair_rank) * (N / 2) + c * 64, kb * GEMM_BK);
+          continue;
+        }
         mbar_arrive_expect_tx(&full_bar[s], a_bytes + b_bytes);
-        const int kb = kb0 + i;
         if (AMODE == A_TMA_K) {
           tma_load_2d(sa, &G.tmA, &full_bar[s], kb * GEMM_BK, m_tile * GEMM_BM);
         } else if (AMODE == A_TMA_MN) {
@@ -189,19 +210,21 @@
             tma_load_2d(sb + c * 8192, &G.tmB, &full_bar[s], G.n_off + c * 64, kb * GEMM_BK);
         }
       }
+      if (PAIR)
+        for (int i = max(0, nkb - kStages); i < nkb; ++i) mbar_wait(&empty_bar[i % kStages], (i / kStages) & 1);
     }
   } else if (warp == 1) {
     if (elect_one()) {
-      const uint32_t idesc = umma_idesc_bf16(GEMM_BM, static_cast<uint32_t>(N),
+      const uint32_t idesc = umma_idesc_bf16(PAIR ? 2 * GEMM_BM : GEMM_BM, static_cast<uint32_t>(N),
                                              (AMODE == A_TMA_MN || AMODE == A_GATHER_MN) ? 1u : 0u,
                                              (BMODE == B_TMA_MN) ? 1u : 0u);
-      for (int i = 0; i < nkb; ++i) {
-        const int s = i % GEMM_STAGES;
-        const uint32_t ph = (i / GEMM_STAGES) & 1;
+      for (int i = 0; i < (mma_cta ? nkb : 0); ++i) {
+        const int s = i % kStages;
+        const uint32_t ph = (i / kStages) & 1;
         mbar_wait(&full_bar[s], ph);
         tc_fence_after();
         if (i == 0) GEMM_STAMP(8);
-        const uint32_t sa = base + s * GEMM_STAGE_BYTES;
+        const uint32_t sa = base + s * kStageBytes;
         const uint32_t sb = sa + GEMM_A_BYTES;
 #pragma unroll
         for (int j = 0; j < GEMM_BK / 16; ++j) {
@@ -210,16 +233,22 @@
           else da = umma_smem_desc(sa + j * 2048, 8192, 1024);
           if (BMODE == B_TMA_K) db = umma_smem_desc(sb + j * 32, 16, 1024);
           else db = umma_smem_desc(sb + j * 2048, 8192, 1024);
-          umma_bf16(tmem_base, da, db, idesc, (i > 0 || j > 0) ? 1u : 0u);
+          if (PAIR) umma_bf16_pair(tmem_base, da, db, idesc, (i > 0 || j > 0) ? 1u : 0u);
+          else umma_bf16(tmem_base, da, db, idesc, (i > 0 || j > 0) ? 1u : 0u);
           if (kColsum)
             umma_bf16(tmem_base + 256, umma_smem_desc(ones + j * 32, 16, 1024),
                       umma_smem_desc(sb + j * 2048 + (cs_c0 >> 6) * 8192, 8192, 1024),
                       umma_idesc_bf16(GEMM_BM, static_cast<uint32_t>(cs_nc), 0u, 1u), (i > 0 || j > 0) ? 1u : 0u);
         }
-        umma_commit(&empty_bar[s]);
-      }
-      umma_commit(tmem_full_bar);
-      GEMM_STAMP(9);
+        if (PAIR) umma_commit_pair(&empty_bar[s], 0x3);
+        else umma_commit(&empty_bar[s]);
+      }
+      if (PAIR) {
+        if (mma_cta && nkb > 0) umma_commit_pair(tmem_full_bar, 0x3);
+      } else {
+        umma_commit(tmem_full_bar);
+      }
+      if (mma_cta) GEMM_STAMP(9);
       if (EPI == EPI_PARTIAL) {
         for (int c = 0; c < N / 32; ++c) {
           mbar_wait(&chunk_bar[c], 0);
@@ -405,8 +434,19 @@
   }
 
   tc_fence_before();
-  __syncthreads();
-  if (warp == 1 && ext_tmem == GEMM_NO_TMEM) tmem_dealloc(tmem_base, kTmemCols);
+  if (PAIR) {
+    cluster_arrive();
+  } else {
+    __syncthreads();
+    if (warp == 1 && ext_tmem == GEMM_NO_TMEM) tmem_dealloc(tmem_base, kTmemCols);
+  }
+  return tmem_base;
+}
+
+MINPPO_DEVINL void gemm_pair_release(uint32_t tmem_base) {
+  cluster_wait();
+  tc_fence_after();
+  if ((threadIdx.x >> 5) == 1) tmem_dealloc2(tmem_base, 512);
 }
 
 template <int EPI>
diff --git a/minppo_b200/learner.py b/minppo_b200/learner.py
--- a/minppo_b200/learner.py
+++ b/minppo_b200/learner.py
@@ -258,6 +258,14 @@
                                                 _stream_ptr(self.device)))
         return out
 
+    @property
+    def dw_path(self) -> dict:
+        out = torch.empty((4,), dtype=torch.int32, device=self.device)
+        with torch.cuda.device(self.device):
+            _lib.check(self.lib.minppo_ctx_read(self._h, 9, _ptr(out), 16, _stream_ptr(self.device)))
+        v = out.cpu().tolist()
+        return {"pairs": bool(v[0]), "grid": v[1], "splits": v[2], "nsplit": v[3]}
+
     def update_host(self, host: "HostBatch") -> np.ndarray:
         host.to_device(self.device)
         ts = TrainState(host.d["params"], host.d["mu"], host.d["nu"], host.d["step"])
```

Result: faster. 51.46 million, median of 6 (+2.7%).
